# ChicyChen/LOCO-Edit

Hardware: AMD Instinct MI355X
Metric: edit-directions/sec (top-5 PMP-Jacobian SVD @256^2) + vT cos-sim vs ref (higher is better)
Workload: dtype bf16x3 (split-bf16 MFMA operands, fp32 accumulate + fp32 storage); 1 GPU; CelebA-HQ DDPM 256x256 top-5 local basis (l_eye-sized mask, L=2400), t=0.6T, 12 power iterations, one GPU; multi_gpu_form=single, probes_total=5, probes_per_gpu=5, kept=5, n_iter=12, mask_L=2400, weights=synthetic seed 0, streams=2

## Files before the change

### include/loco_hip_diag.h

```cpp
#ifndef LOCO_HIP_DIAG_H
#define LOCO_HIP_DIAG_H
#include "loco_hip.h"
#ifdef __cplusplus
extern "C" {
#endif

int  loco_bench_conv(loco_ctx* ctx, int32_t cin, int32_t cout, int32_t H, int32_t W, int32_t B, int32_t mode,
                     int32_t taps, int32_t tile, int32_t iters, float* ms_avg, void* stream);

typedef struct loco_conv_desc {
    int32_t struct_size;
    int32_t Cin, Cout, Hin, Win, B, taps;
    int32_t stride, upsample, zins, mode, cpg;
    int32_t transposed, accumulate, in_arena, pad;
    int32_t Cin2, cot_cpg;
    float   res_scale;
    int32_t st_cpg;
    const float *weight, *bias;
    const float *in, *bias2, *res;
    const float *prim, *sc, *sh, *mr, *gamma, *tst, *tc;
    const float *in2, *w2, *bias2nd;
    const float *cot_d, *cot_prim, *cot_sc, *cot_sh, *cot_mr, *cot_tc;
    float* out;
    const float *st_prim, *st_mr;
// ... 21 lines not shown
    const float *dq, *dk, *dv;
    float* out;
    const float* go;
    float *gq, *gk, *gv;
} loco_attn_desc;
int  loco_debug_attn(loco_ctx* ctx, const loco_attn_desc* desc, char* route, int64_t cap, void* stream);

typedef struct loco_norm_desc {
    int32_t struct_size;
    int32_t op, kind, act, B, C, HW, G, C1, ntA, ntB, accumulate;
    float   eps, base_scale;
    int64_t x_bs, d_bs, base_bs, out_bs, pbs_c, pbs_g, o_bs, t_bs;
    const float *x, *d, *base, *gamma, *beta, *ss_scale, *ss_shift, *sc, *sh, *mr, *tst, *partA, *partB;
    float *o_mr, *o_sc, *o_sh, *o_tst, *o_tc, *out;
} loco_norm_desc;
int  loco_debug_norm(loco_ctx* ctx, const loco_norm_desc* desc, void* stream);

typedef struct loco_gemm_prob {
    const float *A, *B, *A2, *B2, *bias, *colbias, *R;
    float* C;
    int64_t sam, sak, sab, sah;
    int64_t sbk, sbn, sbb, sbh;
    int64_t scm, scn, scb, sch;
    int64_t srb, sab2, sbb2;
    int64_t n_A, n_B, n_A2, n_B2, n_bias, n_colbias, n_R, n_C;
    int32_t M, N, K, batch, batch2;
    float   alpha, beta;
    int32_t pad_;
} loco_gemm_prob;
typedef struct loco_gemm_desc {
    int32_t struct_size;
    int32_t op, act, pad_;
    loco_gemm_prob p[2];
} loco_gemm_desc;
int  loco_debug_gemm(loco_ctx* ctx, const loco_gemm_desc* desc, char* route, int64_t cap, void* stream);

typedef struct loco_pointwise_desc {
    int32_t struct_size;
    int32_t op, kind, act, B, C, T, H, W, n, k, accumulate, cos_first;
    float   eps, scale, t, cv, ce;
    float   f[5];
    int32_t pad_;
    int64_t count, split, in_bs, out_bs, aux_bs, st_bs;
    const float *x, *y, *stats, *gamma, *beta, *base;
    const float *freq, *w0, *b0, *w1, *b1, *add, *add_in;
    const float *src[4];
    const uint8_t *mask, *mask2;
    float *out, *out2, *t_dev;
} loco_pointwise_desc;
int  loco_debug_pointwise(loco_ctx* ctx, const loco_pointwise_desc* desc, void* stream);

int64_t loco_debug_tensor(loco_ctx* ctx, const char* name, float* dst, int64_t cap, void* stream);

#ifdef __cplusplus
}
#endif
#endif
```

### loco-edit_amd/csrc/conv_bf16.hip

```cpp
#include "kernels.h"
#include <cstdio>
#include <cstdlib>

namespace loco {

enum : int { PR_BF16X3 = 0, PR_F16 = 1 };
template <int PR, int TAPS, int MODE> void launch_tile_b(const ConvArgs& a, hipStream_t st);
template <int PR, int MODE> void launch_kcat_b(const ConvArgs& a, hipStream_t st);
template <int PR, int MODE> void launch_pair_b(const ConvArgs& a, hipStream_t st);
void launch_conv_gemm(const ConvArgs& a, hipStream_t st);
template <int PR> void launch_poly_b(const ConvArgs& a, hipStream_t st);
template <int PR> void launch_poly_in_b(const ConvArgs& a, hipStream_t st);

template <int PR>
static void launch_lowp(const ConvArgs& a, int taps, hipStream_t st) {
#ifdef LOCO_DIAG
    if (a.cot_d && (taps != 1 || a.gemm || a.nsplit > 1 || a.Cin2 > 0 || (a.Cout % conv_bf16_tile_couts(a)) != 0 || a.st_kind == ST_TAN || a.st_kind == ST_COT)) {
        fprintf(stderr, "loco: ConvArgs::cot_d on a launch whose epilogue has no norm-cotangent term (taps %d, gemm %d, nsplit %d, Cout %d, st_kind %d)\n",
                taps, a.gemm, a.nsplit, a.Cout, a.st_kind);
        abort();
    }
#endif
    if constexpr (PR == PR_BF16X3) {
        if (taps == 1 && a.gemm) { launch_conv_gemm(a, st); return; }
    }
    if (taps == 9 && a.poly == 2) { launch_poly_in_b<PR>(a, st); return; }
    if (taps == 9 && a.poly) { launch_poly_b<PR>(a, st); return; }
    if (taps == 9 && a.Cin2 > 0) {
        if (a.mode == CM_GN_SILU) launch_kcat_b<PR, CM_GN_SILU>(a, st);
        else if (a.mode == CM_GN_GELU) launch_kcat_b<PR, CM_GN_GELU>(a, st);
        else launch_kcat_b<PR, CM_TAN_SILU>(a, st);
        return;
    }
    if constexpr (PR == PR_BF16X3) {
        if (taps == 9 && a.pair) {
            switch (a.mode) {
                case CM_NONE: launch_pair_b<PR, CM_NONE>(a, st); break;
                case CM_GN_SILU: launch_pair_b<PR, CM_GN_SILU>(a, st); break;
                case CM_TAN_SILU: launch_pair_b<PR, CM_TAN_SILU>(a, st); break;
                default: launch_pair_b<PR, CM_COT_SILU>(a, st); break;
            }
            return;
        }
    }
    if (taps == 9) {
        switch (a.mode) {
            case CM_NONE: launch_tile_b<PR, 9, CM_NONE>(a, st); break;
            case CM_GN_SILU: launch_tile_b<PR, 9, CM_GN_SILU>(a, st); break;
            case CM_GN_GELU: launch_tile_b<PR, 9, CM_GN_GELU>(a, st); break;
            case CM_TAN_SILU: launch_tile_b<PR, 9, CM_TAN_SILU>(a, st); break;
            case CM_COT_SILU: launch_tile_b<PR, 9, CM_COT_SILU>(a, st); break;
            default: launch_tile_b<PR, 9, CM_GN>(a, st); break;
        }
    } else {
        switch (a.mode) {
            case CM_NONE: launch_tile_b<PR, 1, CM_NONE>(a, st); break;
            default: launch_tile_b<PR, 1, CM_GN>(a, st); break;
        }
    }
}
void launch_conv_bf16x3(const ConvArgs& a, int taps, hipStream_t st) { launch_lowp<PR_BF16X3>(a, taps, st); }
void launch_conv_f16(const ConvArgs& a, int taps, hipStream_t st) { launch_lowp<PR_F16>(a, taps, st); }

}
```

### loco-edit_amd/csrc/conv_bf16_kernel.h

```cpp
#pragma once
#include "kernels.h"
#include <cstdlib>
#include <type_traits>

namespace loco {


typedef float f32x16 __attribute__((ext_vector_type(16)));
typedef float f32x4 __attribute__((ext_vector_type(4)));
typedef f32x4 f32x4_u __attribute__((aligned(4)));
typedef float f32x2 __attribute__((ext_vector_type(2)));
typedef f32x2 f32x2_u __attribute__((aligned(4)));
typedef __bf16 bf16x8 __attribute__((ext_vector_type(8)));
typedef _Float16 f16x8 __attribute__((ext_vector_type(8)));
typedef short s16x8 __attribute__((ext_vector_type(8)));

enum : int { PR_BF16X3 = 0, PR_F16 = 1 };

constexpr int BKC = 16;
constexpr bool LIVE_MASK = true;
constexpr bool EARLY_W = true;
constexpr int NDUMMY = 8;

__device__ __forceinline__ float sigmoidf2_(float y) { return __builtin_amdgcn_rcpf(1.0f + __expf(-y)); }
// ... 389 lines not shown
            o0[q] = f32x4{v0[0], v1[0], v0[1], v1[1]};
            o1[q] = f32x4{v0[2], v1[2], v0[3], v1[3]};
        }
        if (accu) {
            f32x4 r0[NP], r1[NP];
#pragma unroll
            for (int q = 0; q < NP; ++q) {
                const unsigned o = (unsigned)(ch0 + h * 32 + q * RSTEP + row0) * out_plane + pix0;
                r0[q] = *reinterpret_cast<const f32x4*>(ob + o);
                r1[q] = *reinterpret_cast<const f32x4*>(ob + o + 4);
            }
#pragma unroll
            for (int q = 0; q < NP; ++q) { o0[q] += r0[q]; o1[q] += r1[q]; }
        }
#pragma unroll
        for (int q = 0; q < NP; ++q) {
            const int co = ch0 + h * 32 + q * RSTEP + row0;
            const unsigned o = (unsigned)co * out_plane + pix0;
            float add = 0.f;
            if (a.bias) add += a.bias[co];
            if (b2) add += b2[co];
            o0[q] += add; o1[q] += add;
            __builtin_nontemporal_store(o0[q], reinterpret_cast<f32x4*>(ob + o));
            __builtin_nontemporal_store(o1[q], reinterpret_cast<f32x4*>(ob + o + 4));
            if (tan_st) {
                const f32x4 va = o0[q], vb = o1[q], xa = xs[q][0], xb = xs[q][1];
                av[(h * NP + q) * 2] = ((va[0] + va[1]) + (va[2] + va[3])) + ((vb[0] + vb[1]) + (vb[2] + vb[3]));
                av[(h * NP + q) * 2 + 1] = (fmaf(xa[0], va[0], xa[1] * va[1]) + fmaf(xa[2], va[2], xa[3] * va[3])) +
                                           (fmaf(xb[0], vb[0], xb[1] * vb[1]) + fmaf(xb[2], vb[2], xb[3] * vb[3]));
            }
        }
    }
    if (tan_st) {
        constexpr int STEPS = rs_steps(NV, 64), LEFT = NV >> STEPS;
        static_assert((NV & (NV - 1)) == 0, "row sums per lane");
        rs_reduce<NV, 1, 64>(av, lane);
        if (lane < (1 << STEPS)) {
            int base = 0;
#pragma unroll
            for (int sb = 0; sb < STEPS; ++sb) base += ((lane >> sb) & 1) * (NV >> (sb + 1));
            const int ntl = (a.Hout * a.Wout) / NT, ntile = 2 * ntl;
            float* const sp = a.st_part + (long)b * C * ntile * 2;
#pragma unroll
            for (int i = 0; i < LEFT; ++i) {
                const int idx = base + i, hq = idx >> 1;
                const int h = hq / NP, q = hq - h * NP;
                const int co = ch0 + h * 32 + q * RSTEP + row0;
                sp[((long)co * ntile + pa * ntl + tile_id) * 2 + (idx & 1)] = av[i];
            }
        }
    }
}

template <int PR, int TAPS, int WM, int WN, int TM, int TN, int MODE, int STG, int PHASE = 0>
__device__ __forceinline__ void conv_lowp_body(const ConvArgs& a, f32x16 (&acc)[TM][TN]) {
    constexpr int NTHR = WM * WN * 64;
    constexpr int HP = halo_pitch<PR>();
    constexpr int RB = rec_bytes<PR>();
    constexpr int NPC = RB / 16;
    constexpr int MT = WM * TM * 32;
    constexpr int NT = WN * TN * 32;
    constexpr bool POLY = (TAPS == 4 && STG == 0), PIN = (TAPS == 4 && STG == 1);
    static_assert(TAPS != 4 || POLY || PIN, "4-tap kernels: the two polyphase forms");
    static_assert(!PIN || (MODE == CM_NONE && PHASE == 0), "polyphase input form: raw");
    constexpr int KS = (TAPS == 9) ? 3 : (TAPS == 4 ? 2 : 1);
    constexpr int HK = (TAPS == 1) ? 1 : 3;
    constexpr int NTS = KS;
    constexpr int NROW = KS;
    static_assert(!POLY || (WM == 2 && TM == 2 && MODE == CM_NONE && PHASE == 0), "polyphase output form: 128 x 256 tile, raw vector staging");
    constexpr bool NEEDP = (MODE == CM_TAN_SILU || MODE == CM_COT_SILU);
    constexpr bool GEN = (STG == 1 || STG == 2);
    constexpr int NITEM = GEN ? (2 * max_halo(NT, TAPS, STG == 2) + NTHR - 1) / NTHR : 1;
    constexpr int WTOT = NTS * MT * NPC;
    constexpr int NWV = (WTOT + NTHR - 1) / NTHR;
    constexpr bool XPF = (TAPS == 9 && STG != 2);
    constexpr int NWB = XPF ? 3 : 2;
    constexpr bool DEEP1 = (TAPS == 1 && STG == 1 && !NEEDP);
    constexpr int DEEP_D = 4;

    extern __shared__ __attribute__((aligned(16))) unsigned char smem_b[];
#ifdef LOCO_DUAL_STAMP
#define LP_STAMP(i) do { if (threadIdx.x == 0 && PHASE == 0) reinterpret_cast<unsigned long long*>(a.partial)[blockIdx.x * 8 + (i)] = __builtin_amdgcn_s_memtime(); } while (0)
#else
#define LP_STAMP(i) do { } while (0)
#endif
    LP_STAMP(0);
    constexpr int WBYTES = NTS * MT * RB;
    unsigned char* const Wsb = smem_b;
    unsigned char* Hsb;
    unsigned char* Ws = smem_b;
    unsigned char* Hs = smem_b;

    const int tid = threadIdx.x;
    const int lane = tid & 63;
    const int wave = tid >> 6;
    const int l31 = lane & 31;
    const int khalf = lane >> 5;
    const int wm = wave / WN, wn = wave % WN;

    const int S = a.stride;
    const int TW = (TAPS == 1 && PHASE == 0 && a.stride == 1 && !a.upsample && !a.zins && (a.Wout & (a.Wout - 1)) == 0)
                       ? (a.Wout < NT ? a.Wout : NT) : (a.Wout < 32 ? a.Wout : 32);
    const int TH = NT / TW;
    const int tiles_x = a.Wout / TW;
    int tile_id, cot_id, zid;
    {
        const int ntile = (a.Hout * a.Wout) / NT, ncot = (a.Cout + MT - 1) / MT, Z = a.B * a.nsplit;
        const int NTC = ntile * ncot, L = blockIdx.x;
        int T = 0;
        if ((ntile & 7) == 0) {
            int q = L >> 3, q2, t8;
            idivmod_small(q, ncot, q2, cot_id);
            idivmod_small(q2, Z, t8, zid);
            tile_id = t8 * 8 + (L & 7);
        } else {
            if ((NTC & 7) == 0) { int q = L >> 3, t8; idivmod_small(q, Z, t8, zid); T = t8 * 8 + (L & 7); }
            else idivmod_small(L, Z, T, zid);
            idivmod_small(T, ntile, cot_id, tile_id);
        }
        tile_id = __builtin_amdgcn_readfirstlane(tile_id);
        cot_id = __builtin_amdgcn_readfirstlane(cot_id);
        zid = __builtin_amdgcn_readfirstlane(zid);
    }
    int ty0_, tx0_;
    idivmod_small(tile_id, tiles_x, ty0_, tx0_);
    const int oy0 = __builtin_amdgcn_readfirstlane(ty0_ * TH);
    const int ox0 = __builtin_amdgcn_readfirstlane(tx0_ * TW);
    const int co0 = cot_id * MT;
    int zb_, zs_;
    idivmod_small(zid, a.nsplit, zb_, zs_);
    const int b = __builtin_amdgcn_readfirstlane(zb_);
    const int split = __builtin_amdgcn_readfirstlane(zs_);

    if constexpr (XPF && PHASE != 2 && EARLY_W) {
        const int nchunks_ = (a.Cin + BKC - 1) / BKC;
        const int cps_ = __builtin_amdgcn_readfirstlane((nchunks_ + a.nsplit - 1) / a.nsplit);
        const int cbeg_ = split * cps_;
        const int cend_ = (cbeg_ + cps_ < nchunks_) ? cbeg_ + cps_ : nchunks_;
        if (cend_ > cbeg_) {
            typedef __attribute__((address_space(3))) unsigned char lds_u8_;
            typedef const __attribute__((address_space(1))) unsigned char glb_u8_;
            const int wpitch_ = (a.Cout + 31) & ~31;
            const unsigned char* wbase0 = reinterpret_cast<const unsigned char*>(a.wb) +
                                          (unsigned)(cbeg_ * TAPS) * ((unsigned)wpitch_ * (unsigned)RB);
#pragma unroll
            for (int st_ = 0; st_ < 2; ++st_)
#pragma unroll
                for (int i = 0; i < NWV; ++i) {
                    int e = tid + i * NTHR;
                    if (e >= WTOT) e = WTOT - 1;
                    const int tap = e / (MT * NPC), rem = e - tap * (MT * NPC);
                    int rec = co0 + rem / NPC;
                    if (rec >= wpitch_) rec = wpitch_ - 1;
                    const unsigned rel = (unsigned)(((st_ * NTS + tap) * wpitch_ + rec) * NPC + (rem % NPC)) * 16u;
                    const int e0 = wave * 64 + i * NTHR;
                    if ((WTOT % NTHR) == 0 || e0 < WTOT)
                        __builtin_amdgcn_global_load_lds((glb_u8_*)(wbase0 + rel), (lds_u8_*)(smem_b + st_ * WBYTES + e0 * 16), 16, 0, 0);
                }
        }
    }
    const int halo_w = (TW - 1) * S + HK;
    const int halo_h = (TH - 1) * S + HK;
    const int halo_sz = halo_h * halo_w;
    int pa_ = 0, pb_ = 0;
    if constexpr (POLY) {
        pa_ = __builtin_amdgcn_readfirstlane(idiv_small(cot_id, a.Cout >> 8));
        pb_ = __builtin_amdgcn_readfirstlane(wm);
    }
    int tap0 = pa_ * halo_w + pb_;
    const int HBYTES = (halo_sz + NDUMMY) * HP;
    Hsb = smem_b + NWB * WBYTES;

    const int LH = (a.upsample || a.zins) ? a.Hin * 2 : a.Hin;
    const int LW = (a.upsample || a.zins) ? a.Win * 2 : a.Win;
    const long in_plane = PIN ? 4L * a.Hin * a.Win : (long)a.Hin * a.Win;

    int ipos[NITEM], ioct[NITEM];
    unsigned ivoff[NITEM];
    bool ival[NITEM];
#pragma unroll
    for (int i = 0; i < NITEM; ++i) {
        int it = tid + i * NTHR;
        int oct, pos;
        idivmod_small(it, halo_sz, oct, pos);
        int off = -1;
// ... 645 lines not shown
                dma_w(cclamp(chunk + dc), r1, Wnxt);
                dma_live = true;
            }
            Ws = Wcur; Hs = Hcur;
            Frag f0, f1;
            load_frag(f0, row, 0);
            if (NTS > 1) load_frag(f1, row, 1);
            __builtin_amdgcn_sched_barrier(0);
            mma_frag(f0);
            __builtin_amdgcn_sched_barrier(0);
            if (NTS > 2) load_frag(f0, row, 2);
            __builtin_amdgcn_sched_barrier(0);
            if (NTS > 1) mma_frag(f1);
            if (st_part >= 0) { Hs = Hnxt; stage_h(cclamp(chunk + 1), st_part); Hs = Hcur; }
            if (MIDLOAD && ld_part >= 0) { pf_live = LIVE_MASK ? (ld_chunk <= clast) : true; prefetch_h(cclamp(ld_chunk), ld_part); pf_live = true; }
            if (NTS > 2) mma_frag(f0);
            __builtin_amdgcn_sched_barrier(0);
            if (MIDLOAD && ld_part >= 0) {
                asm volatile("s_waitcnt vmcnt(%0)" :: "n"(NLD) : "memory");
            } else {
                asm volatile("s_waitcnt vmcnt(0)" ::: "memory");
                if (!MIDLOAD && ld_part >= 0) { pf_live = LIVE_MASK ? (ld_chunk <= clast) : true; prefetch_h(cclamp(ld_chunk), ld_part); pf_live = true; }
            }
            stage_end();
        }
    }
    }

    }

    if constexpr (PHASE == 1) {
        asm volatile("s_waitcnt lgkmcnt(0)" ::: "memory");
        __builtin_amdgcn_s_barrier();
        return;
    }
    LP_STAMP(3);
    if constexpr (POLY) conv_lowp_epilogue_poly<WM, WN, TM, TN>(a, acc, smem_b, cot_id, pa_, oy0, ox0, TW, tile_id, b);
    else conv_lowp_epilogue<WM, WN, TM, TN, (TAPS == 1 && PHASE == 0) ? (EPI_COT1 | EPI_STATS) : EPI_STATS>(a, acc, smem_b, co0, oy0, ox0, TW, tile_id, b, split);
    LP_STAMP(4);
#undef LP_STAMP
}

constexpr int lowp_min_waves(int taps, int nthr) { return (taps == 1 && nthr <= 256) ? 2 : 1; }
template <int TAPS, int WM, int WN, int TM, int TN, int MODE, int STG>
__global__ __launch_bounds__(WM * WN * 64, lowp_min_waves(TAPS, WM * WN * 64)) void conv_mfma_bf16x3(ConvArgs a) {
    f32x16 acc[TM][TN];
    conv_lowp_body<PR_BF16X3, TAPS, WM, WN, TM, TN, MODE, STG>(a, acc);
}
template <int TAPS, int WM, int WN, int TM, int TN, int MODE, int STG>
__global__ __launch_bounds__(WM * WN * 64, lowp_min_waves(TAPS, WM * WN * 64)) void conv_mfma_f16(ConvArgs a) {
    f32x16 acc[TM][TN];
    conv_lowp_body<PR_F16, TAPS, WM, WN, TM, TN, MODE, STG>(a, acc);
}

template <int PR, int WM, int WN, int TM, int TN, int MODE>
__device__ __forceinline__ void conv_lowp_kcat(const ConvArgs& a) {
    f32x16 acc[TM][TN];
    conv_lowp_body<PR, 9, WM, WN, TM, TN, MODE, 0, 1>(a, acc);
    ConvArgs a2 = a;
    a2.in = a.in2; a2.in_bs = a.in2_bs; a2.Cin = a.Cin2; a2.wb = a.wb2; a2.mode = CM_NONE; a2.pad = 0; a2.in_padded = a.in2_padded;
    conv_lowp_body<PR, 1, WM, WN, TM, TN, CM_NONE, 1, 2>(a2, acc);
}
template <int WM, int WN, int TM, int TN, int MODE>
__global__ __launch_bounds__(WM * WN * 64) void conv_kcat_bf16x3(ConvArgs a) { conv_lowp_kcat<PR_BF16X3, WM, WN, TM, TN, MODE>(a); }
template <int WM, int WN, int TM, int TN, int MODE>
__global__ __launch_bounds__(WM * WN * 64) void conv_kcat_f16(ConvArgs a) { conv_lowp_kcat<PR_F16, WM, WN, TM, TN, MODE>(a); }

template <int PR, int TAPS, int WM, int WN, int TM, int TN, int MODE, int STG>
static void launch_one_b2(const ConvArgs& a, hipStream_t st) {
    constexpr int MT = WM * TM * 32, NT = WN * TN * 32;
    constexpr int KS = (TAPS == 9) ? 3 : (TAPS == 4 ? 2 : 1), HK = (TAPS == 1) ? 1 : 3;
    int TW = a.Wout < 32 ? a.Wout : 32;
    int TH = NT / TW;
    int halo_w = (TW - 1) * a.stride + HK, halo_h = (TH - 1) * a.stride + HK;
    const int nwb = (TAPS == 9 && STG != 2) ? 3 : 2;
    size_t lds = (size_t)nwb * KS * MT * rec_bytes<PR>() + 2 * ((size_t)halo_w * halo_h + NDUMMY) * halo_pitch<PR>();
    const size_t stage_bytes = (size_t)WM * 32 * NT * 4;
    if (lds < stage_bytes) lds = stage_bytes;
    dim3 grid(((a.Hout * a.Wout) / NT) * ((a.Cout + MT - 1) / MT) * a.B * a.nsplit);
    void (*kern)(ConvArgs);
    if constexpr (PR == PR_F16) kern = &conv_mfma_f16<TAPS, WM, WN, TM, TN, MODE, STG>;
    else kern = &conv_mfma_bf16x3<TAPS, WM, WN, TM, TN, MODE, STG>;
    if (lds > 64 * 1024) {
        static DeviceOnce once;
        if (first_on_device(once)) {
            (void)hipFuncSetAttribute(reinterpret_cast<const void*>(kern), hipFuncAttributeMaxDynamicSharedMemorySize,
                                      160 * 1024);
        }
    }
    hipLaunchKernelGGL(kern, grid, dim3(WM * WN * 64), lds, st, a);
}

template <int PR, int TAPS, int WM, int WN, int TM, int TN, int MODE>
static void launch_one_b(const ConvArgs& a, hipStream_t st) {
    const bool general = a.stride != 1 || a.upsample || a.zins || (a.Cin % BKC) != 0 || !a.in_padded;
    if constexpr (MODE == CM_NONE) {
        if (a.stride == 2) launch_one_b2<PR, TAPS, WM, WN, TM, TN, MODE, 2>(a, st);
        else if (TAPS == 9 && !general) launch_one_b2<PR, TAPS, WM, WN, TM, TN, MODE, 0>(a, st);
        else launch_one_b2<PR, TAPS, WM, WN, TM, TN, MODE, 1>(a, st);
        return;
    }
    if constexpr (MODE == CM_GN_SILU || MODE == CM_TAN_SILU || MODE == CM_GN_GELU) {
        if (general) { launch_one_b2<PR, TAPS, WM, WN, TM, TN, MODE, 1>(a, st); return; }
    }
    launch_one_b2<PR, TAPS, WM, WN, TM, TN, MODE, 0>(a, st);
}


template <int PR, int MODE>
void launch_kcat_b(const ConvArgs& a, hipStream_t st) {
    constexpr int WM = 2, WN = 4, TM = 2, TN = 2, MT = 128, NT = 256;
    const int TW = a.Wout < 32 ? a.Wout : 32, TH = NT / TW;
    size_t lds = (size_t)3 * 3 * MT * rec_bytes<PR>() + 2 * ((size_t)(TW + 2) * (TH + 2) + NDUMMY) * halo_pitch<PR>();
    dim3 grid(((a.Hout * a.Wout) / NT) * ((a.Cout + MT - 1) / MT) * a.B * a.nsplit);
    void (*kern)(ConvArgs);
    if constexpr (PR == PR_F16) kern = &conv_kcat_f16<WM, WN, TM, TN, MODE>;
    else kern = &conv_kcat_bf16x3<WM, WN, TM, TN, MODE>;
    static DeviceOnce once;
    if (first_on_device(once))
        (void)hipFuncSetAttribute(reinterpret_cast<const void*>(kern), hipFuncAttributeMaxDynamicSharedMemorySize, 160 * 1024);
    hipLaunchKernelGGL(kern, grid, dim3(WM * WN * 64), lds, st, a);
}

template <int PR>
void launch_poly_b(const ConvArgs& a, hipStream_t st) {
    ConvArgs v = a;
    v.Cout = 4 * a.Cout; v.Hout = a.Hin; v.Wout = a.Win;
    v.upsample = 0; v.zins = 0; v.stride = 1; v.pad = 1; v.nsplit = 1;
    launch_one_b2<PR, 4, 2, 4, 2, 2, CM_NONE, 0>(v, st);
}

template <int PR>
void launch_poly_in_b(const ConvArgs& a, hipStream_t st) {
    ConvArgs v = a;
    v.Cin = 4 * a.Cin; v.Hin = a.Hin / 2; v.Win = a.Win / 2;
    v.upsample = 0; v.zins = 0; v.stride = 1; v.pad = 1; v.nsplit = 1;
    launch_one_b2<PR, 4, 2, 4, 2, 2, CM_NONE, 1>(v, st);
}

template <int PR, int TAPS, int MODE>
void launch_tile_b(const ConvArgs& a, hipStream_t st) {
    switch (a.tile) {
        case 5:
            launch_one_b<PR, TAPS, 2, 4, 2, 2, MODE>(a, st);
            break;
        case 0: launch_one_b<PR, TAPS, 2, 2, 2, 2, MODE>(a, st); break;
        case 1: launch_one_b<PR, TAPS, 4, 1, 1, 2, MODE>(a, st); break;
        case 2: launch_one_b<PR, TAPS, 1, 4, 1, 1, MODE>(a, st); break;
        default: launch_one_b<PR, TAPS, 2, 2, 1, 1, MODE>(a, st); break;
    }
}


}
```

### loco-edit_amd/csrc/conv_plan.hip

```cpp
#include "kernels.h"
#include <cstdio>
#include <cstdlib>

namespace loco {

constexpr int BKC = 16;
constexpr int BKF = 8;

static const int kMT[6] = {128, 128, 32, 64, 128, 128}, kNT[6] = {128, 64, 128, 64, 256, 256};

static int env_int(const char* name, int dflt) {
    const char* e = getenv(name);
    return e ? atoi(e) : dflt;
}
static int pick_tile(int Cout, int HW) {
    if (HW >= 128) return Cout > 32 ? 0 : 2;
    return Cout > 64 ? 1 : 3;
}

static int conv_pick_nsplit(int Cin, int Cout, int Hout, int Wout, int B) {
    const int t = pick_tile(Cout, Hout * Wout);
    long blocks = (long)((Hout * Wout) / kNT[t]) * ((Cout + kMT[t] - 1) / kMT[t]) * B;
    int nchunks = (Cin + BKF - 1) / BKF;
    if (blocks >= 384 || nchunks < 8) return 1;
// ... 33 lines not shown
    static const bool on = env_int("LOCO_POLYPHASE", 1) != 0;
    if (!on || e.prec < 1 || taps != 9 || a.mode != CM_NONE || !(a.upsample || a.zins) || a.stride != 1) return false;
    if (!(e.prec == 2 ? a.wph : a.wpb) || !a.in_padded || a.res || a.Cin2 > 0 || a.cot_d) return false;
    if (a.upsample ? a.pad != 1 : (a.pad != 1 && a.pad != 2)) return false;
    if ((a.Cin % BKC) != 0 || (a.Cout % 128) != 0 || a.B < 2) return false;
    if (a.Hin * a.Win < 4096 || a.Win < 32 || (a.Win % 32) != 0 || (a.Hin % 8) != 0) return false;
    return a.Hout == 2 * a.Hin && a.Wout == 2 * a.Win;
}
static bool conv_poly_in_ok(const ConvEnv& e, const ConvArgs& a, int taps) {
    static const bool on = env_int("LOCO_POLYPHASE", 1) != 0;
    if (!on || e.prec < 1 || taps != 9 || a.mode != CM_NONE || !a.pool2 || a.upsample || a.zins || a.stride != 1 || a.pad != 1) return false;
    if (!(e.prec == 2 ? a.wqh : a.wqb) || a.res || a.bias2 || a.Cin2 > 0 || a.cot_d) return false;
    if ((a.Cin % BKC) != 0 || (a.Cout % 128) != 0 || a.B < 2 || ((a.Hin | a.Win) & 1)) return false;
    if (a.Hout * a.Wout < 4096 || a.Wout < 32 || (a.Wout % 32) != 0 || (a.Hout % 8) != 0) return false;
    return a.Hin == 2 * a.Hout && a.Win == 2 * a.Wout;
}

static int conv_bf16_pick_nsplit(int Cin, int Cout, int Hout, int Wout, int B, int chip_share, int taps, int lanes) {
    const int HW = Hout * Wout;
    int t = conv_bf16_pick_tile(Cout, HW, B, -1);
    if (t == 4) t = 5;
    if (taps == 1 && t == 5 && B >= 2 && HW <= kTile0MaxHW) t = 0;
    long blocks = (long)(HW / kNT[t]) * ((Cout + kMT[t] - 1) / kMT[t]) * B;
    int nchunks = (Cin + BKC - 1) / BKC;
    int target = chip_share > 1 ? 256 / chip_share : (lanes == 2 ? 240 : 256);
    if (target < 32) target = 32;
    if (blocks >= target / 2 || nchunks < 8) return 1;
    int want = (int)(target / blocks);
    int maxs = nchunks / 4;
    if (want > maxs) want = maxs;
    if (want > 32) want = 32;
    return want < 1 ? 1 : want;
}

static bool conv_lowp_can_kcat(const ConvArgs& a) {
    static const bool on = env_int("LOCO_KCAT", 1) != 0;
    return on && a.Cin2 > 0 && a.nsplit == 1 && bf16_tile_of(a) == 5 && a.stride == 1 && !a.upsample && !a.zins && a.pad == 1 &&
           (a.Cin % BKC) == 0 && (a.Cin2 % BKC) == 0 && a.in_padded &&
           (a.mode == CM_GN_SILU || a.mode == CM_GN_GELU || a.mode == CM_TAN_SILU);
}
static bool conv_lowp_can_fuse_stats(const ConvArgs& a) {
    return a.nsplit <= 1 && !a.gemm && (a.Cout % conv_bf16_tile_couts(a)) == 0;
}

static bool conv_pair_ok(const ConvArgs& a) {
    static const bool on = env_int("LOCO_CONV_PAIR", 1) != 0;
    if (!on || a.poly || a.Hout * a.Wout < 16384 || a.taps != 9 || a.Cin2 > 0 || a.nsplit != 1 || a.stride != 1 || a.upsample || a.zins ||
        a.pad != 1 || !a.in_padded || (a.Cin % (2 * BKC)) != 0 || (a.Cout % 128) != 0 || (a.Wout % 32) != 0 || (a.Hout % 8) != 0)
        return false;
    if (!(a.mode == CM_NONE || a.mode == CM_GN_SILU || a.mode == CM_TAN_SILU || a.mode == CM_COT_SILU)) return false;
    return a.tile == 5;
}

static ConvArgs conv_shift_batch(const ConvArgs& a, int nb) {
    ConvArgs t = a;
    t.B = a.B - nb;
    t.in += (long)nb * a.in_bs; t.out += (long)nb * a.out_bs;
    if (t.prim) t.prim += (long)nb * a.prim_bs;
    if (t.bias2) t.bias2 += (long)nb * a.bias2_bs;
    if (t.res) t.res += (long)nb * a.res_bs;
    if (t.sc) { t.sc += (long)nb * a.scsh_bs; t.sh += (long)nb * a.scsh_bs; }
    if (t.mr) t.mr += (long)nb * a.mr_bs;
    if (t.tst) t.tst += (long)nb * a.tst_bs;
    if (t.tc) t.tc += (long)nb * a.tc_bs;
    if (t.in2) t.in2 += (long)nb * a.in2_bs;
    if (t.cot_d) { t.cot_d += (long)nb * a.cot_d_bs; t.cot_tc += (long)nb * a.cot_tc_bs; }
    if (t.st_part) t.st_part += (long)nb * a.Cout * ((a.Hout * a.Wout) / conv_bf16_tile_pixels(a)) * 2;
    return t;
}

static void conv_gemm_plan(ConvArgs& a) {
    static const bool on = env_int("LOCO_CONV_GEMM", 1) != 0;
    a.gemm = 0;
    const long HW = (long)a.Hout * a.Wout;
    if (!on || a.stride != 1 || a.upsample || a.zins || (a.Cin % BKC) != 0 || a.Cin < 320 || (HW % 256) != 0 || (a.Wout % 16) != 0 ||
        a.Cout < 128 || !a.partial || a.Cin2 > 0 || !(a.mode == CM_NONE || a.mode == CM_GN) || a.cot_d)
        return;
    {
        const int TW = a.Wout < 32 ? a.Wout : 32;
        if ((256 % TW) != 0 || (a.Wout % TW) != 0 || (a.Hout % (256 / TW)) != 0) return;
    }
    static const int all_shapes = env_int("LOCO_GEMM_ALL", 0);
    if (!all_shapes && !(a.Cout >= 640 && (a.Cout >= 4 * a.Cin || a.Cin >= 2560))) return;
    const int pad256 = (a.Cout + 255) / 256 * 256;
    const int tm = (pad256 * 10 <= a.Cout * 11) ? 4 : 2;
    const int mt = 64 * tm;
    const long tiles = (HW / 256) * ((a.Cout + mt - 1) / mt) * a.B;
    const size_t rec_floats = (size_t)a.B * a.Cin * HW;
    int ns = 1;
    if (tiles < 192) {
        const int nchunks = a.Cin / BKC;
        ns = (int)((256 + tiles - 1) / tiles);
        if (ns > 8) ns = 8;
        while (ns > 1 && nchunks / ns < 8) --ns;
        while (ns > 1 && (size_t)ns * a.B * a.Cout * HW + rec_floats > a.partial_floats) --ns;
    }
    if ((ns > 1 ? (size_t)ns * a.B * a.Cout * HW : 0) + rec_floats > a.partial_floats) return;
    a.gemm = 1; a.gemm_tm = tm; a.nsplit = ns;
}

void conv_plan_family(ConvArgs& a, int prec) {
    if (prec == 1 && a.taps == 1) conv_gemm_plan(a);
}

void conv_plan_tile_pair(ConvArgs& a, int prec, int tile_override) {
    a.tile = tile_for(a, prec, tile_override);
// ... 59 lines not shown
}

ConvPlan plan_conv(const ConvEnv& e, const ConvArgs& a0, int taps, const StatAsk* q, const ConvArgs* sc) {
    ConvPlan p;
    ConvArgs a = a0;
    a.taps = taps;
    a.gemm = 0;
    a.poly = 0;
    if (a.pool2) {
        if (conv_poly_in_ok(e, a, taps)) a.poly = 2;
        else {
            p.pool_after = true; p.pool_out = a.out; p.pool_out_bs = a.out_bs; p.pool_acc = a.accumulate;
            a.out = a.pool_tmp; a.out_bs = a.pool_tmp_bs; a.Hout = a.Hin; a.Wout = a.Win; a.accumulate = 0; a.pool2 = 0;
        }
    }
    if (sc) {
        ConvArgs t = a;
        t.nsplit = e.prec >= 1 ? conv_bf16_pick_nsplit(a.Cin, a.Cout, a.Hout, a.Wout, a.B, e.chip_share, 9, e.lanes) : 2;
        t.in2 = sc->in; t.in2_bs = sc->in_bs; t.Cin2 = sc->Cin;
        const long per_probe = (long)((a.Hout * a.Wout) / 256) * ((a.Cout + 127) / 128);
        if (e.prec >= 1 && taps == 9 && !short_tail(per_probe, a.B) && !a.bias2 && conv_lowp_can_kcat(t)) {
            a.in2 = sc->in; a.in2_bs = sc->in_bs; a.Cin2 = sc->Cin; a.in2_padded = sc->in_padded;
            a.wb2 = e.prec == 2 ? sc->wh : sc->wb;
            a.bias2 = sc->bias; a.bias2_bs = 0;
            a.res = nullptr;
        } else {
            p.sc_first = true;
            a.res = sc->out; a.res_bs = sc->out_bs;
        }
    }
    if (e.prec == 2) a.wb = a.wh;
    a.no_deep = e.deep1 ? 0 : 1;
    a.nsplit = e.prec >= 1 ? conv_bf16_pick_nsplit(a.Cin, a.Cout, a.Hout, a.Wout, a.B, e.chip_share, taps, e.lanes)
                           : conv_pick_nsplit(a.Cin, a.Cout, a.Hout, a.Wout, a.B);
    if (a.cot_d) {
        ConvArgs t = a;
        t.tile = bf16_tile_of(t);
        const long per_probe = (long)((a.Hout * a.Wout) / conv_bf16_tile_pixels(t)) * ((a.Cout + 127) / 128);
        p.cot = e.prec >= 1 && taps == 1 && a.nsplit == 1 && !short_tail(per_probe, a.B) && conv_lowp_can_fuse_stats(t);
        if (!p.cot) { a.cot_d = nullptr; a.cot_d_bs = 0; a.cot_sx = nullptr; a.cot_tc = nullptr; a.cot_tc_bs = 0; }
    }
    while (a.nsplit > 1 && (size_t)a.nsplit * a.B * a.Cout * a.Hout * a.Wout > e.partial_floats) a.nsplit >>= 1;
    if (a.nsplit < 1) a.nsplit = 1;
    a.partial = e.partial;
    a.partial_floats = e.partial_floats;
    if (!a.poly && conv_poly_ok(e, a, taps)) a.poly = 1;
    if (a.poly == 1) { a.nsplit = 1; a.wb = e.prec == 2 ? a.wph : a.wpb; }
    if (a.poly == 2) { a.nsplit = 1; a.wb = e.prec == 2 ? a.wqh : a.wqb; }
    conv_plan_family(a, e.prec);
    a.tile = tile_for(a, e.prec, -1);
    int split = 1;
    const int tail = e.prec >= 1 && a.nsplit == 1 && a.B >= 2 && !a.gemm && !a.poly ? tail_split(a, e.partial_floats, &split) : 0;
    const bool want = q && q->kind != ST_NONE && e.prec >= 1 && e.fuse_stats;
    if (!tail) {
        p.l[0] = plan_launch(e, q, want, a, 0, a.B, &p.keep_ntile);
        return p;
    }
    const bool per_part = want && q->norm && (q->kind == ST_FWD || (e.fuse_lin && (a.Hout * a.Wout) % 4 == 0));
    p.stats_all = !per_part && q && q->kind != ST_NONE && q->norm;
    const StatAsk* ql = per_part ? q : nullptr;
    const int nb = a.B - tail;
    ConvArgs m = a, t = conv_shift_batch(a, nb);
    m.B = nb;
    t.nsplit = split;
    p.nl = 2;
    p.l[0] = plan_launch(e, ql, want, m, 0, a.B, &p.keep_ntile);
    p.l[1] = plan_launch(e, ql, want, t, nb, a.B, &p.keep_ntile);
    return p;
}

void polyphase_fold(int kind, int nin, int nout, const float* w, long so, long si, long st, float* out) {
    static const int sel[3][2][2][3] = {
        {{{1, 0, 0}, {0, 1, 1}}, {{1, 1, 0}, {0, 0, 1}}},
        {{{1, 0, 0}, {0, 0, 1}}, {{0, 1, 0}, {0, 0, 0}}},
        {{{0, 0, 0}, {0, 1, 0}}, {{1, 0, 0}, {0, 0, 1}}}};
    const long V = 4L * nout;
    for (int i = 0; i < nin; ++i)
        for (int pa = 0; pa < 2; ++pa)
            for (int pb = 0; pb < 2; ++pb)
                for (int ty = 0; ty < 2; ++ty)
                    for (int tx = 0; tx < 2; ++tx)
                        for (int o = 0; o < nout; ++o) {
                            double acc = 0.0;
                            for (int ky = 0; ky < 3; ++ky)
                                for (int kx = 0; kx < 3; ++kx)
                                    if (sel[kind][pa][ty][ky] && sel[kind][pb][tx][kx]) acc += (double)w[o * so + i * si + (3 * ky + kx) * st];
                            out[((long)i * 4 + 2 * ty + tx) * V + polyphase_vcout(nout, pa, pb, o)] = (float)acc;
                        }
}

void polyphase_fold_in(int nin, int nout, const float* w, long so, long si, long st, float* out, int noutP) {
    for (int p = 0; p < 2; ++p)
        for (int q = 0; q < 2; ++q)
            for (int i = 0; i < nin; ++i)
                for (int ty = 0; ty < 2; ++ty)
                    for (int tx = 0; tx < 2; ++tx) {
                        const int m = 2 * ty + 1 - p, n = 2 * tx + 1 - q;
                        for (int o = 0; o < nout; ++o) {
                            double acc = 0.0;
                            for (int a = 0; a < 2; ++a)
                                for (int b = 0; b < 2; ++b) {
                                    const int ky = m - a, kx = n - b;
                                    if (ky >= 0 && ky < 3 && kx >= 0 && kx < 3) acc += (double)w[o * so + i * si + (3 * ky + kx) * st];
                                }
                            out[((((long)(2 * p + q) * nin + i) * 4) + 2 * ty + tx) * noutP + o] = (float)acc;
                        }
                    }
}

const char* conv_variant_name(const ConvArgs& a, int taps, int prec) {
    static const char* tiles[6] = {"2,2,2,2", "4,1,1,2", "1,4,1,1", "2,2,1,1", "2,2,2,4", "2,4,2,2"};
    static char names[3][2][6][6][56];
    static char others[3][3][6][40];
    const int mode = (a.mode < 0 || a.mode > 5) ? 2 : a.mode;
    const char* other = nullptr;
    int k = 0, v = mode;
    if (prec && taps == 9 && a.poly) {
        static const char* pn[2][3] = {{"", "conv_mfma_bf16x3<4,2,4,2,2,0>", "conv_mfma_f16<4,2,4,2,2,0>"},
                                       {"", "conv_mfma_bf16x3<4,2,4,2,2,0>+pool", "conv_mfma_f16<4,2,4,2,2,0>+pool"}};
        return pn[a.poly == 2][prec];
    }
    if (prec && taps == 9 && a.Cin2 > 0) other = prec == 1 ? "conv_kcat_bf16x3<2,4,2,2,%d>" : "conv_kcat_f16<2,4,2,2,%d>";
    else if (prec == 1 && taps == 1 && a.gemm) { k = 1; other = "conv_gemm_bf16x3<%d>"; v = a.gemm_tm; }
    else if (prec == 1 && taps == 9 && a.pair) { k = 2; other = "conv_pair_bf16x3<%d>"; }
    if (other) {
        char* n = others[k][prec][v];
        if (!n[0]) snprintf(n, 40, other, v);
        return n;
    }
    int t = a.tile;
    if (t < 0 || t > 5) t = 0;
    int m = mode;
    if (taps != 9 && m != CM_NONE) m = CM_GN;
    if (!prec && m == CM_GN_GELU) m = CM_GN_SILU;
    char* n = names[prec][taps == 9 ? 0 : 1][t][m];
    static const char* kn[3] = {"conv_mfma_f32", "conv_mfma_bf16x3", "conv_mfma_f16"};
    if (!n[0]) snprintf(n, 56, "%s<%d,%s,%d>", kn[prec], taps, tiles[t], m);
    return n;
}

}
```

### loco-edit_amd/csrc/conv_plan_text.h

```cpp
#pragma once
#include "kernels.h"
#include <cstdio>
#include <string>

namespace loco {

inline const char* stat_route_name(int r) {
    static const char* names[5] = {"none", "epi", "splitk", "alone", "keep"};
    return r >= 0 && r < 5 ? names[r] : "?";
}

inline void conv_plan_text(const ConvPlan& p, int taps, int prec, std::string& out) {
    char line[384];
    for (int li = 0; li < p.nl; ++li) {
        const ConvLaunch& l = p.l[li];
        const ConvArgs& y = l.args;
        snprintf(line, sizeof(line),
                 "launch=%d part=0 kernel=%s tile=%d nsplit=%d B=%d s0=%d gemm=%d gemm_tm=%d pair=%d Cin2=%d sc_first=%d cot=%d "
                 "stats=%s ntile=%d\n",
                 li, conv_variant_name(y, taps, prec), y.tile, y.nsplit, y.B, l.s0, y.gemm, y.gemm ? y.gemm_tm : 0, y.pair, y.Cin2,
                 p.sc_first ? 1 : 0, p.cot ? 1 : 0, stat_route_name(l.stats), l.ntile);
        out += line;
    }
    snprintf(line, sizeof(line), "stats_all=%d keep_ntile=%d\n", p.stats_all ? 1 : 0, p.keep_ntile);
    out += line;
}

}
```

### loco-edit_amd/csrc/engine.hip

```cpp
#include <algorithm>
#include <array>
#include <cmath>
#include <cstdio>
#include <cstdlib>
#include <cstring>

#include "conv_plan_text.h"
#include "engine_internal.h"

using namespace loco;
using namespace loco::eng;

namespace loco {
namespace eng {

int upload(loco_ctx* c, float** dst, const std::vector<float>& h) {
    if (dalloc(c, dst, h.size() ? h.size() : 1)) return -1;
    HIPCHK(c, hipMemcpy(*dst, h.data(), h.size() * sizeof(float), hipMemcpyHostToDevice));
    return 0;
}

namespace {
struct Pass {
    loco_ctx* c;
    hipStream_t st;
    int B;
    float* arena;
    float* stats;
    TView T(int id) const { return tview(c, arena, id); }
};

static void drop_graphs(loco_ctx* c) {
    for (auto& kv : c->fwd_graphs) {
        if (kv.second.exec) (void)hipGraphExecDestroy(kv.second.exec);
        if (kv.second.graph) (void)hipGraphDestroy(kv.second.graph);
    }
    c->fwd_graphs.clear();
}
inline unsigned char* gemm_ws_get(loco_ctx* c, size_t need, hipStream_t st) {
    const int l = c->lane;
    if (c->gemm_ws_bytes[l] >= need) return c->gemm_ws[l];
    hipStreamCaptureStatus cs = hipStreamCaptureStatusNone;
    if (hipStreamIsCapturing(st, &cs) != hipSuccess || cs != hipStreamCaptureStatusNone) return nullptr;
    if (c->gemm_ws[l]) {
        (void)hipDeviceSynchronize();
        drop_graphs(c);
        (void)hipFree(c->gemm_ws[l]);
        c->bytes -= c->gemm_ws_bytes[l];
        c->gemm_ws[l] = nullptr; c->gemm_ws_bytes[l] = 0;
    }
    void* p = nullptr;
    if (hipMalloc(&p, need) != hipSuccess) { (void)hipGetLastError(); return nullptr; }
    c->gemm_ws[l] = static_cast<unsigned char*>(p); c->gemm_ws_bytes[l] = need; c->bytes += need;
    return c->gemm_ws[l];
}
inline void attn_note(loco_ctx* c, const char* kernel, const GemmArgs* g = nullptr) {
    if (!c->attn_log) return;
    char line[192];
    if (g) snprintf(line, sizeof(line), "kernel=%s M=%d N=%d K=%d batch=%d heads=%d kcat=%d\n", kernel, g->M, g->N, g->K, g->batch,
                    g->batch2 > 0 ? g->batch2 : 1, g->A2 ? 1 : 0);
    else snprintf(line, sizeof(line), "kernel=%s\n", kernel);
    *c->attn_log += line;
}
inline bool attn_gemm_rec(const loco_ctx* c, const GemmArgs& g) { return c->prec >= 1 && c->gemm_lowp && gemm_rec_eligible(g); }
inline void attn_gemm_f32(loco_ctx* c, const GemmArgs& g, hipStream_t st) { attn_note(c, "gemm_f32", &g); launch_gemm(g, st); }
inline void attn_gemm(loco_ctx* c, const GemmArgs& g, hipStream_t st) {
    if (attn_gemm_rec(c, g)) {
        if (unsigned char* ws = gemm_ws_get(c, gemm_rec_ws_bytes(g), st)) { attn_note(c, "gemm_rec", &g); launch_gemm_rec(g, ws, st); return; }
    }
    if (c->prec >= 1 && c->gemm_lowp && gemm_prefers_bf16x3(g)) { attn_note(c, "gemm_bf16x3", &g); launch_gemm_bf16x3(g, st); }
    else attn_gemm_f32(c, g, st);
}
inline void attn_gemm_pair(loco_ctx* c, const GemmArgs& g0, const GemmArgs& g1, hipStream_t st) {
    auto f32 = [&](const GemmArgs& g) { return !attn_gemm_rec(c, g) && !(c->prec >= 1 && c->gemm_lowp && gemm_prefers_bf16x3(g)); };
    if (!f32(g0) || !f32(g1)) { attn_gemm(c, g0, st); attn_gemm(c, g1, st); return; }
    attn_note(c, "gemm_f32", &g0); attn_note(c, "gemm_f32", &g1);
    launch_gemm_pair(g0, g1, st);
}
inline void attn_softmax_rows(loco_ctx* c, float* S, long rows, int T, hipStream_t st, int B, long bs) {
    attn_note(c, "softmax_rows"); launch_softmax_rows(S, rows, T, st, B, bs);
}
inline void attn_softmax_jac(loco_ctx* c, float* dS, const float* P, long rows, int T, float scale, hipStream_t st, int B, long bs) {
    attn_note(c, "softmax_jac"); launch_softmax_jac(dS, P, rows, T, rows, scale, st, B, bs);
}
}

NS nstats(const loco_ctx* c, float* base, const NormP& n) {
    NS s;
    s.sc = base + n.soff; s.sh = s.sc + n.C; s.mr = s.sh + n.C; s.tst = s.mr + 2 * c->cfg.gn_groups;
    s.tc = s.tst + 2 * c->cfg.gn_groups;
    return s;
}

static void stats_standalone(loco_ctx* c, const StatReq& rq, const float* x, long xbs, int B, int HW, int s0, hipStream_t st) {
    const NormP& n = *rq.n;
    const long SB = c->prog->stats_per_sample;
    const int G = c->cfg.gn_groups;
    if (rq.kind == ST_FWD) {
        NS s = nstats(c, rq.stats + (long)s0 * SB, n);
        launch_gn_stats(x, xbs, B, n.C, HW, G, eps_of(c, n), n.gamma, n.beta, s.mr, s.sc, s.sh, SB, c->red, st, rq.ss_scale,
                        rq.ss_shift);
    } else {
        NS sp = nstats(c, c->statsP, n);
        NS stt = nstats(c, rq.stats + (long)s0 * SB, n);
        launch_gn_tstats(x, xbs, rq.prim, 0, B, n.C, HW, G, sp.sc, sp.sh, sp.mr, 0, 0, rq.kind == ST_TAN ? 0 : 1, stt.tst,
                         stt.tc, SB, c->red, st, c->cfg.act);
    }
}

bool run_conv(loco_ctx* c, const ConvArgs& a0, int taps, hipStream_t st, const StatReq* rq, const ConvArgs* second) {
    const size_t span = (size_t)c->cfg.max_batch * c->prog->per_sample;
    auto padded = [&](const float* p) { return (p >= c->arenaP && p < c->arenaP + span) || (p >= c->arenaT && p < c->arenaT + span); };
    ConvArgs a = a0, sc;
    a.act = c->cfg.act;
    if (a.mode == CM_GN_SILU && c->cfg.act == ACT_GELU) a.mode = CM_GN_GELU;
    a.in_padded = padded(a.in);
    if (second) { sc = *second; sc.in_padded = padded(sc.in); }
    ConvEnv e;
    e.prec = c->prec; e.chip_share = c->chip_share; e.lanes = c->lanes_active; e.lane_s0 = c->lane_s0;
    e.partial = c->partial; e.partial_floats = c->partial_floats; e.stpart = c->stpart; e.stpart_floats = c->stpart_floats;
    e.fuse_stats = c->fuse_stats; e.fuse_lin = c->fuse_lin; e.deep1 = c->deep1; e.max_batch = c->cfg.max_batch;
    StatAsk q;
    if (rq) {
        q.kind = rq->kind; q.norm = rq->n != nullptr; q.prim = rq->prim; q.keep = rq->keep; q.keep_floats = rq->keep_floats;
        if (rq->n && rq->n->sx_off >= 0 && c->sxcache) q.sx = c->sxcache + rq->n->sx_off;
    }
    const ConvPlan p = plan_conv(e, a, taps, rq ? &q : nullptr, second ? &sc : nullptr);
    if (p.sc_first) run_conv(c, *second, 1, st);
    if (c->plan_log) conv_plan_text(p, taps, c->prec, *c->plan_log);
    if (rq && rq->kind != ST_NONE && rq->n) rq->n->ready = true;
    if (rq && rq->keep_ntile) *rq->keep_ntile = p.keep_ntile;
    const int HWo = a.Hout * a.Wout, Gn = c->cfg.gn_groups;
    const long SBs = c->prog->stats_per_sample;
    auto timed = [&](const char* name, double flops, const ConvArgs& y, auto&& launch) {
        loco_ctx::ProfRec r;
        if (c->prof_on) {
            r.name = name; r.flops = flops;
            r.cin = y.Cin; r.cout = y.Cout; r.h = y.Hout; r.b = y.B; r.ns = y.nsplit; r.mode = y.mode; r.taps = taps;
            r.e0 = c->next_event(); r.e1 = c->next_event();
            (void)hipEventRecord(r.e0, st);
        }
        launch();
        if (c->prof_on) { (void)hipEventRecord(r.e1, st); c->prof.push_back(r); }
    };
    for (int li = 0; li < p.nl; ++li) {
        const ConvLaunch& l = p.l[li];
        const ConvArgs& x = l.args;
        double flops = 2.0 * (x.Cin * taps + x.Cin2) * x.Cout * (double)x.Hout * x.Wout * x.B;
        if (x.zins) flops *= 0.25;
        if (x.poly == 2) flops *= 4.0;
        timed(c->prof_on ? conv_variant_name(x, taps, c->prec) : nullptr, flops, x, [&] {
            if (c->prec == 1) launch_conv_bf16x3(x, taps, st);
            else if (c->prec == 2) launch_conv_f16(x, taps, st);
            else launch_conv(x, taps, st);
        });
        if (x.nsplit > 1) {
            timed("conv_splitk_reduce", 0.0, x, [&] {
                if (l.stats != SR_SPLITK) { launch_conv_splitk_reduce(x, st); return; }
                const NormP& n = *rq->n;
                NS sp = nstats(c, c->statsP, n);
                NS so = nstats(c, rq->stats + (long)l.s0 * SBs, n);
                launch_conv_splitk_reduce_stats(x, rq->kind, Gn, eps_of(c, n), n.gamma, n.beta, so.mr, so.sc, so.sh, SBs, rq->ss_scale,
                                                rq->ss_shift, rq->prim, sp.sc, sp.sh, sp.mr, so.tst, so.tc, SBs, c->red, st);
            });
        }
        if (l.stats == SR_ALONE) stats_standalone(c, *rq, x.out, x.out_bs, x.B, HWo, l.s0, st);
        if (l.stats == SR_EPI) {
            const NormP& n = *rq->n;
            NS so = nstats(c, rq->stats + (long)l.s0 * SBs, n);
            if (rq->kind != ST_FWD) {
                NS sp = nstats(c, c->statsP, n);
                launch_gn_lin_fused_finalize(rq->kind, x.st_part, n.C, l.ntile, nullptr, 0, x.B, n.C, HWo, Gn, sp.mr, so.tst, so.tc,
                                             SBs, st);
            } else {
                launch_gn_fused_finalize(x.st_part, l.ntile, x.B, n.C, HWo, Gn, eps_of(c, n), n.gamma, n.beta, so.mr, so.sc, so.sh,
                                         SBs, rq->ss_scale, rq->ss_shift, st);
            }
        }
    }
    if (p.stats_all) stats_standalone(c, *rq, a.out, a.out_bs, a.B, HWo, 0, st);
    if (p.pool_after)
// ... 281 lines not shown
        attn_gemm_pair(c, attn_values(s, IMAGE, k, 0, SG, s.bS, gq, s.bq, s.HS, 0.f),
                       attn_keys(s, q, 0, s.HS, SG, s.bS, gk, s.bq), s.st);
        return;
    }
    attn_gemm(c, attn_keys(s, oG, s.bo, s.OS, SP, 0, gv, s.bq), s.st);
    if (s.Lt) attn_gemm_f32(c, attn_scores(s, TEXT, oG, s.bo, s.OS, s.vt, 0, SG, s.bS, 1.f, 0.f), s.st);
    attn_gemm(c, attn_scores(s, IMAGE, oG, s.bo, s.OS, v, 0, SG, s.bS, 1.f, 0.f), s.st);
    attn_softmax_jac(c, SG, SP, (long)s.NH * s.T, s.Tk, s.scale, s.st, s.B, s.bS);
    attn_gemm(c, attn_values(s, IMAGE, k, 0, SG, s.bS, gq, s.bq, s.HS, 0.f), s.st);
    if (s.Lt) attn_gemm_f32(c, attn_values(s, TEXT, s.kt, 0, SG, s.bS, gq, s.bq, s.HS, 1.f), s.st);
    attn_gemm(c, attn_keys(s, q, 0, s.HS, SG, s.bS, gk, s.bq), s.st);
}

}
}

namespace {

void lin1x1(loco_ctx* c, const ConvP& w, bool dgrad, const TView& in, const TView& out, int B, hipStream_t st,
            const float* bias = nullptr, const float* res = nullptr, const StatReq* rq = nullptr) {
    ConvArgs a = conv_args(in, w, dgrad, out, B, 1);
    a.bias = bias; a.res = res; a.res_bs = res ? out.bs : 0;
    run_conv(c, a, 1, st, rq);
}

void need_fwd_stats(const Pass& p, NormP& n, int tid, bool cat = false) {
    loco_ctx* c = p.c;
    if (!n.ready && !(cat && cat_fused_stats(c, n, tid, p.stats, p.B, p.st))) {
        const TView x = p.T(tid);
        NS s = nstats(c, p.stats, n);
        launch_gn_stats(x, x.bs, p.B, n.C, x.H * x.W, c->cfg.gn_groups, eps_of(c, n), n.gamma, n.beta, s.mr, s.sc, s.sh,
                        c->prog->stats_per_sample, c->red, p.st);
    }
    n.ready = false;
}

void lin_stats(const Pass& p, const NormP& n, int kind, const TView& d, const float* x) {
    loco_ctx* c = p.c;
    NS sp = nstats(c, c->statsP, n);
    NS stt = nstats(c, p.stats, n);
    launch_gn_tstats(d, d.bs, x, 0, p.B, n.C, d.H * d.W, c->cfg.gn_groups, sp.sc, sp.sh, sp.mr, 0, 0, kind, stt.tst,
                     stt.tc, c->prog->stats_per_sample, c->red, p.st, kind ? c->cfg.act : 0);
}
void need_tan_stats(const Pass& p, NormP& n, int tid, bool cat = false) {
    loco_ctx* c = p.c;
    if (!n.ready && !(cat && cat_fused_tstats(c, n, tid, p.B, p.st))) lin_stats(p, n, 0, p.T(tid), tview(c, c->arenaP, tid));
    n.ready = false;
}
void need_cot_stats(const Pass& p, NormP& n, const TView& d, const float* x) {
    if (!n.ready) lin_stats(p, n, 1, d, x);
    n.ready = false;
}
void gn_lin_apply(const Pass& p, const NormP& n, int kind, const TView& d, const float* x, const float* base, float* out,
                  int accumulate = 0, float base_scale = 1.0f) {
    loco_ctx* c = p.c;
    NS sp = nstats(c, c->statsP, n);
    NS stt = nstats(c, p.stats, n);
    launch_gn_apply(kind, d, d.bs, x, 0, base, base ? d.bs : 0, out, d.bs, accumulate, p.B, d.C, d.H * d.W, c->cfg.gn_groups,
                    sp.sc, sp.sh, sp.mr, 0, 0, stt.tst, c->prog->stats_per_sample, p.st, kind == 2 || kind == 5 ? c->cfg.act : 0,
                    base_scale);
}
void set_tan(loco_ctx* c, ConvArgs& a, const NormP& n, const float* prim) {
    NS sp = nstats(c, c->statsP, n);
    NS stt = nstats(c, c->statsT, n);
    a.mode = CM_TAN_SILU; a.prim = prim; a.prim_bs = 0;
    a.sc = sp.sc; a.sh = sp.sh; a.scsh_bs = 0; a.mr = sp.mr; a.mr_bs = 0; a.gamma_ = n.gamma;
    a.tst = stt.tst; a.tst_bs = c->prog->stats_per_sample; a.cpg = n.C / c->cfg.gn_groups;
    a.tc = stt.tc; a.tc_bs = c->prog->stats_per_sample;
    a.sx = (n.sx_off >= 0 && c->sxcache) ? c->sxcache + n.sx_off : nullptr;
}

constexpr size_t RED_BYTES = (size_t)4 << 20;

int forward_pass(loco_ctx* c, const float* x, float t, int B, float* arena, float* stats, hipStream_t st,
                 const float* t_ptr = nullptr, int op_hi = -1, const float* dh = nullptr) {
    const loco_unet_cfg& cfg = c->cfg;
    const Pass p{c, st, B, arena, stats};
    const long PS = c->prog->per_sample, SB = c->prog->stats_per_sample;
    auto T = [&](int id) { return p.T(id); };
    const TView xv = tview_in(x, c->prog->n_in, cfg.in_channels, cfg.resolution, cfg.resolution);
    clear_ready(c);
    auto next_fwd = [&](int tid) { return req_fwd_of(c, tid, stats); };
    auto gn_prologue = [&](ConvArgs& a, int mode, const NS& s) { a.mode = mode; a.sc = s.sc; a.sh = s.sh; a.scsh_bs = SB; };
    if (cfg.arch < 2) {
        launch_temb(t, cfg.ch, cfg.ch * 4, c->wts->freq, c->wts->td0w, c->wts->td0b, c->wts->td1w, c->wts->td1b, c->tact, st, cfg.arch == 1,
                    c->has_cond ? c->cond_add : nullptr, t_ptr, cfg.act, c->has_tcond ? c->cond_in : nullptr);
        launch_temb_proj(c->tact, cfg.ch * 4, c->wts->tp_w, c->wts->tp_b, (int)c->wts->tproj_total, c->tproj, st);
    }
    const int op_end = op_hi >= 0 ? op_hi : (int)c->ops.size() - 1;
    for (int oi = 0; oi <= op_end; ++oi) {
        Op& op = c->ops[oi];
        const Tens& to = c->tens[op.out];
        switch (op.kind) {
            case OP_CONV_IN: case OP_CONV: {
                ConvArgs a = conv_args(op.kind == OP_CONV_IN ? xv : T(op.in), op.conv, false, T(op.out), B, op.ksize);
                a.bias = op.conv.bias;
                const StatReq rq = next_fwd(op.out);
                run_conv(c, a, op.ksize == 1 ? 1 : 9, st, &rq);
                break;
            }
            case OP_RES: {
                const Tens& ti = c->tens[op.in];
                need_fwd_stats(p, op.n1, op.in, true);
                NS s1 = nstats(c, stats, op.n1);
                if (op.updown == 1) {
                    launch_gn_apply(4, nullptr, 0, T(op.in), PS, nullptr, 0, T(op.a1), PS, 0, B, ti.C, ti.H * ti.W,
                                    cfg.gn_groups, s1.sc, s1.sh, s1.mr, SB, SB, nullptr, 0, st, cfg.act);
                    launch_pool2x2_sum(T(op.a1), PS, T(op.ap), PS, 0, B, ti.C, to.H, to.W, st, 0.25f);
                    launch_pool2x2_sum(T(op.in), PS, T(op.xu), PS, 0, B, ti.C, to.H, to.W, st, 0.25f);
                } else if (op.updown == 2) {
                    launch_upsample2x(T(op.in), PS, T(op.xu), PS, 0, 1.0f, B, ti.C, ti.H, ti.W, st);
                }
                ConvArgs a = conv_args(op.updown == 1 ? T(op.ap) : T(op.in), op.c1, false, T(op.h1), B, 3);
// ... 47 lines not shown
                    lin1x1(c, op.xproj, false, T(op.xo), T(op.out), B, st, op.xproj.bias, T(op.xmid), &rqx);
                }
                break;
            }
            case OP_XFMR: {
                if (!c->has_ctx) { c->err = "this architecture has cross-attention stages: call loco_set_context first"; return -1; }
                const int C = to.C, HW = to.H * to.W;
                auto X = [&](int i) { return T(op.xt[i]); };
                need_fwd_stats(p, op.n1, op.in);
                {
                    ConvArgs a = conv_args(T(op.in), op.pj_in, false, X(X_H0), B, 1);
                    a.bias = op.pj_in.bias;
                    gn_prologue(a, CM_GN, nstats(c, stats, op.n1));
                    run_conv(c, a, 1, st);
                }
                const XA xa = xa_of(c, op, B, st);
                launch_ln_fwd(X(X_H0), PS, B, C, HW, op.lng[0], op.lnb[0], 1e-5f, X(X_A1), PS, X(X_LN1), PS, st);
                lin1x1(c, op.qkvc, false, X(X_A1), X(X_QKV), B, st);
                attn_forward(attn_of(c, op, B, st, arena, PS));
                lin1x1(c, op.to_out1, false, X(X_O), X(X_H1), B, st, op.to_out1.bias, X(X_H0));
                launch_ln_fwd(X(X_H1), PS, B, C, HW, op.lng[1], op.lnb[1], 1e-5f, X(X_A2), PS, X(X_LN2), PS, st);
                lin1x1(c, op.xqc, false, X(X_A2), X(X_XQ), B, st);
                xa_forward(xa, X(X_XQ), X(X_XS), X(X_XO));
                lin1x1(c, op.to_out2, false, X(X_XO), X(X_H2), B, st, op.to_out2.bias, X(X_H1));
                launch_ln_fwd(X(X_H2), PS, B, C, HW, op.lng[2], op.lnb[2], 1e-5f, X(X_A3), PS, X(X_LN3), PS, st);
                lin1x1(c, op.ff1, false, X(X_A3), X(X_F), B, st, op.ff1.bias);
                launch_geglu(0, X(X_F), PS, nullptr, B, 4L * C * HW, X(X_GG), PS, st);
                lin1x1(c, op.ff2, false, X(X_GG), X(X_H3), B, st, op.ff2.bias, X(X_H2));
                const StatReq rq = next_fwd(op.out);
                lin1x1(c, op.pj_out, false, X(X_H3), T(op.out), B, st, op.pj_out.bias, T(op.in), &rq);
                break;
            }
            case OP_DOWN: case OP_UP: {
                ConvArgs a = conv_args(T(op.in), op.conv, false, T(op.out), B, 3);
                a.bias = op.conv.bias;
                if (op.kind == OP_DOWN) { a.stride = 2; a.pad = op.sym_down ? 1 : 0; } else { a.upsample = 1; }
                const StatReq rq = next_fwd(op.out);
                run_conv(c, a, 9, st, &rq);
                break;
            }
            case OP_OUT: {
                need_fwd_stats(p, op.n1, op.in);
                ConvArgs a = conv_args(T(op.in), op.conv, false, T(op.out), B, 3);
                a.bias = op.conv.bias;
                gn_prologue(a, CM_GN_SILU, nstats(c, stats, op.n1));
                run_conv(c, a, 9, st);
                break;
            }
        }
    }
    return 0;
}

int tangent_pass(loco_ctx* c, const float* V, int B, hipStream_t st, int op_lo = 0, int op_hi = -1) {
    const loco_unet_cfg& cfg = c->cfg;
    const long PS = c->prog->per_sample;
    const Pass p{c, st, B, c->arenaT, c->statsT};
    auto TP = [&](int id) { return tview(c, c->arenaP, id); };
    auto TT = [&](int id) { return p.T(id); };
    const TView Vv = tview_in(V, c->prog->n_in, cfg.in_channels, cfg.resolution, cfg.resolution);
    clear_ready(c);
    auto next_tan = [&](int tid) {
        StatReq r = req_lin(c, ST_TAN, consumer_norm(c, tid), TP(tid));
        Tens& t = c->tens[tid];
        if (t.cat_of >= 0 && t.keep && c->fuse_lin) {
            r.kind = ST_TAN; r.stats = c->statsT; r.prim = TP(tid);
            r.keep = t.keep; r.keep_floats = t.keep_floats; r.keep_ntile = &t.keep_ntile;
        }
        return r;
    };
    const int op_end = op_hi >= 0 ? op_hi : (int)c->ops.size() - 1;
    for (int oi = op_lo; oi <= op_end; ++oi) {
        Op& op = c->ops[oi];
        const Tens& to = c->tens[op.out];
        switch (op.kind) {
            case OP_CONV_IN: case OP_CONV: {
                const ConvArgs a = conv_args(op.kind == OP_CONV_IN ? Vv : TT(op.in), op.conv, false, TT(op.out), B, op.ksize);
                const StatReq rq = next_tan(op.out);
                run_conv(c, a, op.ksize == 1 ? 1 : 9, st, &rq);
                break;
            }
            case OP_RES: {
                const Tens& ti = c->tens[op.in];
                need_tan_stats(p, op.n1, op.in, true);
                if (op.updown == 1) {
                    gn_lin_apply(p, op.n1, 5, TT(op.in), TP(op.in), nullptr, TT(op.a1));
                    launch_pool2x2_sum(TT(op.a1), PS, TT(op.ap), PS, 0, B, ti.C, to.H, to.W, st, 0.25f);
                    launch_pool2x2_sum(TT(op.in), PS, TT(op.xu), PS, 0, B, ti.C, to.H, to.W, st, 0.25f);
                } else if (op.updown == 2) {
                    launch_upsample2x(TT(op.in), PS, TT(op.xu), PS, 0, 1.0f, B, ti.C, ti.H, ti.W, st);
                }
                ConvArgs a = conv_args(op.updown == 1 ? TT(op.ap) : TT(op.in), op.c1, false, TT(op.h1), B, 3);
                if (op.updown != 1) { set_tan(c, a, op.n1, TP(op.in)); a.upsample = op.updown == 2; }
                {
                    const StatReq rq2 = req_lin(c, ST_TAN, &op.n2, TP(op.h1));
                    run_conv(c, a, 9, st, &rq2);
                    op.n2.ready = false;
                }
                const TView xin = op.updown ? TT(op.xu) : TT(op.in);
                ConvArgs n{};
                if (op.has_nin) n = conv_args(xin, op.nin, false, TT(op.out), B, 1);
                ConvArgs b = conv_args(TT(op.h1), op.c2, false, TT(op.out), B, 3);
                b.res = xin; b.res_bs = PS;
                b.res_scale = op.has_nin ? 1.f : c->prog->res_scale;
                set_tan(c, b, op.n2, TP(op.h1));
                const StatReq rq = next_tan(op.out);
// ... 6 lines not shown
                gn_lin_apply(p, op.n1, 1, TT(op.in), TP(op.in), nullptr, TT(op.hn));
                lin1x1(c, op.qkvc, false, TT(op.hn), TT(op.qkv), B, st);
                attn_tangent(attn_of(c, op, B, st));
                {
                    const StatReq rq = next_tan(so);
                    lin1x1(c, op.proj, false, TT(op.o), TT(so), B, st, nullptr, TT(op.in), &rq);
                }
                if (op.has_x) {
                    const XA x = xa_of(c, op, B, st);
                    need_tan_stats(p, op.nx, op.xmid);
                    gn_lin_apply(p, op.nx, 1, TT(op.xmid), TP(op.xmid), nullptr, TT(op.xhn));
                    lin1x1(c, op.xqc, false, TT(op.xhn), TT(op.xq), B, st);
                    xa_linear(x, TT(op.xq), op.xK, op.xV, TP(op.xS), TT(op.xS), TT(op.xo));
                    const StatReq rqx = next_tan(op.out);
                    lin1x1(c, op.xproj, false, TT(op.xo), TT(op.out), B, st, nullptr, TT(op.xmid), &rqx);
                }
                break;
            }
            case OP_XFMR: {
                const int C = to.C, HW = to.H * to.W;
                auto XP = [&](int i) { return TP(op.xt[i]); };
                auto XT_ = [&](int i) { return TT(op.xt[i]); };
                need_tan_stats(p, op.n1, op.in);
                gn_lin_apply(p, op.n1, 1, TT(op.in), TP(op.in), nullptr, XT_(X_G0));
                lin1x1(c, op.pj_in, false, XT_(X_G0), XT_(X_H0), B, st);
                const XA xa = xa_of(c, op, B, st);
                launch_ln_tan(XT_(X_H0), PS, XP(X_H0), XP(X_LN1), B, C, HW, op.lng[0], XT_(X_A1), PS, st);
                lin1x1(c, op.qkvc, false, XT_(X_A1), XT_(X_QKV), B, st);
                attn_tangent(attn_of(c, op, B, st));
                lin1x1(c, op.to_out1, false, XT_(X_O), XT_(X_H1), B, st, nullptr, XT_(X_H0));
                launch_ln_tan(XT_(X_H1), PS, XP(X_H1), XP(X_LN2), B, C, HW, op.lng[1], XT_(X_A2), PS, st);
                lin1x1(c, op.xqc, false, XT_(X_A2), XT_(X_XQ), B, st);
                xa_linear(xa, XT_(X_XQ), op.xK, op.xV, XP(X_XS), XT_(X_XS), XT_(X_XO));
                lin1x1(c, op.to_out2, false, XT_(X_XO), XT_(X_H2), B, st, nullptr, XT_(X_H1));
                launch_ln_tan(XT_(X_H2), PS, XP(X_H2), XP(X_LN3), B, C, HW, op.lng[2], XT_(X_A3), PS, st);
                lin1x1(c, op.ff1, false, XT_(X_A3), XT_(X_F), B, st);
                launch_geglu(1, XT_(X_F), PS, XP(X_F), B, 4L * C * HW, XT_(X_GG), PS, st);
                lin1x1(c, op.ff2, false, XT_(X_GG), XT_(X_H3), B, st, nullptr, XT_(X_H2));
                const StatReq rq = next_tan(op.out);
                lin1x1(c, op.pj_out, false, XT_(X_H3), TT(op.out), B, st, nullptr, TT(op.in), &rq);
                break;
            }
            case OP_DOWN: case OP_UP: {
                ConvArgs a = conv_args(TT(op.in), op.conv, false, TT(op.out), B, 3);
                if (op.kind == OP_DOWN) { a.stride = 2; a.pad = op.sym_down ? 1 : 0; } else { a.upsample = 1; }
                const StatReq rq = next_tan(op.out);
                run_conv(c, a, 9, st, &rq);
                break;
            }
            case OP_OUT: {
                need_tan_stats(p, op.n1, op.in);
                ConvArgs a = conv_args(TT(op.in), op.conv, false, TT(op.out), B, 3);
                set_tan(c, a, op.n1, TP(op.in));
                run_conv(c, a, 9, st);
                break;
            }
        }
    }
    return 0;
}

int cotangent_pass(loco_ctx* c, const float* ge, const float* gx0, float* Aout, int B, hipStream_t st, int op_lo = 0,
                   int op_hi = -1) {
    const loco_unet_cfg& cfg = c->cfg;
    const long PS = c->prog->per_sample;
    const Pass p{c, st, B, c->arenaT, c->statsT};
    auto TP = [&](int id) { return tview(c, c->arenaP, id); };
    auto TG = [&](int id) { return p.T(id); };
    auto GO = [&](const Op& o) {
        const Tens& t = c->tens[o.out];
        return o.out == c->prog->eps_t ? tview_in(ge, c->prog->n_out, t.C, t.H, t.W) : TG(o.out);
    };
    const TView Av{Aout, c->prog->n_in, cfg.in_channels, cfg.resolution, cfg.resolution};
    clear_ready(c);
    for (int oi = op_hi >= 0 ? op_hi : (int)c->ops.size() - 1; oi >= op_lo; --oi) {
        Op& op = c->ops[oi];
        const Tens& to = c->tens[op.out];
        const int acc = op.in_is_skip ? 1 : 0;
        switch (op.kind) {
            case OP_OUT: {
                const ConvArgs a = conv_args(GO(op), op.conv, true, TG(op.a1), B, 3);
                {
                    const StatReq rq = req_lin(c, ST_COT, &op.n1, TP(op.in));
                    run_conv(c, a, 9, st, &rq);
                    op.n1.ready = false;
                }
                gn_lin_apply(p, op.n1, 2, TG(op.a1), TP(op.in), nullptr, TG(op.in));
                break;
            }
            case OP_UP: {
                ConvArgs a = conv_args(TG(op.out), op.conv, true, TG(op.in), B, 3);
                a.pool2 = 1; a.pool_tmp = TG(op.up); a.pool_tmp_bs = PS;
                run_conv(c, a, 9, st);
                break;
            }
            case OP_DOWN: {
                ConvArgs a = conv_args(TG(op.out), op.conv, true, TG(op.in), B, 3);
                a.zins = 1; a.pad = op.sym_down ? 1 : 2; a.accumulate = acc;
                run_conv(c, a, 9, st);
                break;
            }
            case OP_RES: {
                const Tens& ti = c->tens[op.in];
                {
                    const ConvArgs a = conv_args(TG(op.out), op.c2, true, TG(op.h1), B, 3);
                    const StatReq rq2 = req_lin(c, ST_COT, &op.n2, TP(op.h1));
                    run_conv(c, a, 9, st, &rq2);
                    op.n2.ready = false;
                }
                ConvArgs b = conv_args(TG(op.h1), op.c1, true, TG(op.updown == 0 ? op.a1 : op.updown == 1 ? op.ap : op.xu), B, 3);
                set_tan(c, b, op.n2, TP(op.h1));
                b.mode = CM_COT_SILU;
                if (op.updown == 0) {
                    const StatReq rq1 = req_lin(c, ST_COT, &op.n1, TP(op.in));
                    run_conv(c, b, 9, st, &rq1);
                } else if (op.updown == 1) {
                    run_conv(c, b, 9, st);
                    launch_upsample2x(TG(op.ap), PS, TG(op.a1), PS, 0, 0.25f, B, ti.C, to.H, to.W, st);
                } else {
                    run_conv(c, b, 9, st);
                    launch_pool2x2_sum(TG(op.xu), PS, TG(op.a1), PS, 0, B, ti.C, ti.H, ti.W, st);
                }
                need_cot_stats(p, op.n1, TG(op.a1), TP(op.in));
                bool cot_in_epilogue = false;
                if (op.has_nin) {
                    ConvArgs n = conv_args(TG(op.out), op.nin, true, TG(op.in), B, 1);
                    n.accumulate = acc;
                    if (op.updown == 0 && c->prec >= 1 && c->fuse_cot && op.n1.sx_off >= 0 && c->sxcache) {
                        n.cot_d = TG(op.a1); n.cot_d_bs = PS; n.cot_sx = c->sxcache + op.n1.sx_off;
                        n.cot_tc = nstats(c, c->statsT, op.n1).tc; n.cot_tc_bs = c->prog->stats_per_sample;
                    }
                    cot_in_epilogue = run_conv(c, n, 1, st);
                }
                if (op.updown == 0) {
                    if (cot_in_epilogue) {  }
                    else if (op.has_nin) gn_lin_apply(p, op.n1, 2, TG(op.a1), TP(op.in), nullptr, TG(op.in), 1);
                    else
                        gn_lin_apply(p, op.n1, 2, TG(op.a1), TP(op.in), TG(op.out), TG(op.in), acc, c->prog->res_scale);
                } else {
                    gn_lin_apply(p, op.n1, 2, TG(op.a1), TP(op.in), nullptr, TG(op.in), acc);
// ... 133 lines not shown
    c->cfg = *cfg;
    c->prog = std::move(prog);
    const size_t MB = (size_t)cfg->max_batch;
    {
        float *p0 = nullptr, *p1 = nullptr;
        if (dalloc(c, &p0, MB * c->prog->per_sample + 128) || dalloc(c, &p1, MB * c->prog->per_sample + 128)) return -1;
        c->arenaP = p0 + 64; c->arenaT = p1 + 64;
    }
    if (dalloc(c, &c->statsP, MB * c->prog->stats_per_sample) || dalloc(c, &c->statsT, MB * c->prog->stats_per_sample)) return -1;
    if (dalloc(c, &c->red, RED_BYTES) || dalloc(c, &c->red2, RED_BYTES)) return -1;
    if (alloc_state(c)) return -1;
    {
        c->stpart_floats = MB * (size_t)(c->prog->max_tensor / 64 + 1) * 2;
        if (dalloc(c, &c->stpart, c->stpart_floats) || dalloc(c, &c->stpart2, c->stpart_floats)) return -1;
        const char* e = getenv("LOCO_FUSE_STATS");
        c->fuse_stats = !(e && atoi(e) == 0);
        e = getenv("LOCO_FUSE_LIN");
        c->fuse_lin = !(e && atoi(e) == 0);
        e = getenv("LOCO_FUSE_COT");
        c->fuse_cot = !(e && atoi(e) == 0) && cfg->act == ACT_SILU;
        e = getenv("LOCO_DEEP1");
        c->deep1 = !(e && atoi(e) == 0);
        e = getenv("LOCO_FUSE_XATTN");
        c->fuse_xattn = !(e && atoi(e) == 0);
        const char* fa = getenv("LOCO_FLASH_ATTN");
        c->flash_attn = !(fa && atoi(fa) == 0);
        if (dalloc(c, &c->attn_delta, MB * (size_t)c->prog->attn_dmax)) return -1;
    }
    c->partial_floats = (size_t)64 << 20;
    if (dalloc(c, &c->partial, c->partial_floats)) return -1;
    if (dalloc(c, &c->xin_buf, MB * c->prog->n_in) || dalloc(c, &c->t_dev, 4)) return -1;
    if (dalloc(c, &c->eps_buf, MB * c->prog->n_out) || dalloc(c, &c->gx0, MB * c->prog->n_in) || dalloc(c, &c->ge, MB * c->prog->n_out))
        return -1;
    c->n_ws = std::max((long)c->prog->n_in, (long)c->prog->n_h);
    if (dalloc(c, &c->tmpA, (size_t)64 * c->n_ws)) return -1;
    if (dalloc(c, &c->G, 64 * 64) || dalloc(c, &c->Q, 64 * 64) || dalloc(c, &c->W, SOLVER_W_GATE + 1)) return -1;
    {
        size_t nblk = ((size_t)c->n_ws + 255) / 256;
        if (dalloc(c, &c->gscratch, nblk * 64 * 64 + 4096)) return -1;
    }
    if (dalloc(c, &c->kry[0], KRY_STATE) || dalloc(c, &c->kry[1], KRY_STATE)) return -1;
    if (dalloc(c, &c->alphas, 256) || dalloc(c, &c->cond_add, (size_t)cfg->ch * 4)) return -1;
    if (dalloc(c, &c->cond_in, (size_t)cfg->ch)) return -1;
    {
        float2* sx0 = nullptr;
        if (dalloc(c, &sx0, (size_t)c->prog->sx_total + 64)) return -1;
        c->sxcache = sx0 + 32;
    }
    {
        const char* e = getenv("LOCO_PRECISION");
        c->prec = (e && std::string(e) == "f32") ? 0 : (e && std::string(e) == "f16") ? 2 : 1;
    }
    if (dalloc(c, &c->mask2, (size_t)c->prog->n_out)) return -1;
    if (dalloc(c, &c->mask, (size_t)c->prog->n_out) || dalloc(c, &c->mask_idx, (size_t)c->prog->n_out) ||
        dalloc(c, &c->mask_L_dev, 4)) return -1;
    HIPCHK(c, hipEventCreate(&c->ev0));
    HIPCHK(c, hipEventCreate(&c->ev1));
    {
        const char* e = getenv("LOCO_STREAMS");
        c->n_streams = (e && atoi(e) == 2) ? 2 : 1;
        HIPCHK(c, hipStreamCreateWithFlags(&c->st2, hipStreamNonBlocking));
        HIPCHK(c, hipStreamCreateWithFlags(&c->cap_st, hipStreamNonBlocking));
        const char* gl = getenv("LOCO_GEMM_LOWP");
        if (gl) c->gemm_lowp = atoi(gl) != 0;
        const char* gr = getenv("LOCO_GRAPH");
        c->graph_on = gr && atoi(gr) == 1;
        HIPCHK(c, hipEventCreateWithFlags(&c->ev_fork, hipEventDisableTiming));
        HIPCHK(c, hipEventCreateWithFlags(&c->ev_join, hipEventDisableTiming));
    }
    return 0;
}

}

extern "C" {

const char* loco_version(void) { return "loco_hip 0.2 (gfx950; conv arithmetic: f32 MFMA | bf16x3 split-bf16 MFMA | f16 MFMA)"; }

int loco_device_count(void) {
    int n = 0;
    if (hipGetDeviceCount(&n) != hipSuccess) return 0;
    return n;
}

int loco_create(const loco_unet_cfg* cfg, loco_ctx** out) {
    if (!cfg || !out) return -2;
    loco_ctx* c = new loco_ctx();
    *out = c;
    if (cfg->struct_size != (int32_t)sizeof(loco_unet_cfg)) {
        c->err = "loco_unet_cfg.struct_size = " + std::to_string(cfg->struct_size) + ", this library expects " +
                 std::to_string(sizeof(loco_unet_cfg)) + " (binding and library built from different headers)";
        return -2;
    }
    auto prog = std::make_shared<Program>();
    if (const int rc = build_program(*cfg, prog.get(), &c->err)) return rc;
    for (const ParamDecl& d : prog->params) c->params[d.name].shape = d.shape;
    c->wts = std::make_shared<Weights>();
    c->wts->op.resize(prog->ops.size());
    return create_ctx(c, cfg, std::move(prog));
}

int loco_fork(loco_ctx* parent, int32_t max_batch, loco_ctx** out) {
    if (!parent || !out) return -2;
    *out = nullptr;
    if (finalize_params(parent)) return -3;
    loco_ctx* root = parent->weights_of ? parent->weights_of : parent;
// ... 196 lines not shown
                    void* stream) {
    return loco_pmp_primal_tap(c, x, t, at, mask, use_et, 0, stream);
}

static int pmp_primal_at(loco_ctx* c, const float* x, float t, float at, const uint8_t* mask, int32_t use_et, int32_t tap, const float* dh,
                         void* stream) {
    if (tap < 0 || tap > 2) { c->err = "loco_pmp_primal_tap: tap must be 0 (x_t -> x0 / eps), 1 (encoder, x_t -> h) or 2 (decoder, h -> eps)"; return -2; }
    if (tap && tap_refuse(c, "loco_pmp_primal_tap")) return -2;
    if (tap == 1 && mask) { c->err = "loco_pmp_primal_tap: the encoder tap (x_t -> h) takes no mask: h has no pixel positions to select"; return -2; }
    if (finalize_params(c)) return -3;
    if (dh) {
        const Op& op = c->ops[c->prog->h_last_op];
        if (op.kind != OP_RES || op.has_nin || op.updown) { c->err = "loco_pmp_primal_tap_dh: the tap op is not an identity-shortcut ResBlock"; return -2; }
    }
    if (tap == 1) use_et = 1;
    if (c->prog->n_out != c->prog->n_in && !use_et) {
        c->err = "loco_pmp_primal: a network whose output size differs from its input has no x0 combination; use_et = 1 "
                 "(raw network Jacobian)";
        return -2;
    }
    hipStream_t st = (hipStream_t)stream;
    const int op_lo = tap == 2 ? c->prog->h_last_op + 1 : 0, op_hi = tap == 1 ? c->prog->h_last_op : (int)c->ops.size() - 1;
    if (forward_pass(c, x, t, 1, c->arenaP, c->statsP, st, nullptr, tap == 1 ? op_hi : -1, dh)) return -1;
    c->primal_B = 1;
    if (c->prec >= 1) {
        for (int oi = op_lo; oi <= op_hi; ++oi) {
            Op& op = c->ops[oi];
            if (op.kind != OP_RES && op.kind != OP_OUT) continue;
            const Tens& ti = c->tens[op.in];
            const int HW = ti.H * ti.W, G = c->cfg.gn_groups;
            NS s1 = nstats(c, c->statsP, op.n1);
            launch_gn_cache(c->arenaP + ti.off, op.n1.C, HW, op.n1.C / G, s1.sc, s1.sh, s1.mr,
                            c->sxcache + op.n1.sx_off, st, c->cfg.act);
            if (op.kind == OP_RES) {
                const Tens& th = c->tens[op.h1];
                NS s2 = nstats(c, c->statsP, op.n2);
                launch_gn_cache(c->arenaP + th.off, op.n2.C, th.H * th.W, op.n2.C / G, s2.sc, s2.sh, s2.mr,
                                c->sxcache + op.n2.sx_off, st, c->cfg.act);
            }
        }
    }
    if (use_et) { c->p_cv = 0.f; c->p_ce = 1.f; }
    else { c->p_cv = 1.0f / std::sqrt(at); c->p_ce = -std::sqrt(1.0f - at) / std::sqrt(at); }
    if (tap == 2) c->p_cv = 0.f;
    c->tap = tap;
    c->has_mask = (mask != nullptr);
    c->has_mask2 = false;
    c->mask_L = tap == 1 ? c->prog->n_h : c->prog->n_out;
    if (mask) {
        HIPCHK(c, hipMemcpyAsync(c->mask, mask, (size_t)c->prog->n_out, hipMemcpyDeviceToDevice, st));
        launch_mask_compact(c->mask, c->prog->n_out, c->mask_idx, c->mask_L_dev, st);
        c->mask_L = -1;
        c->mask_stream = st;
    }
    HIPCHK(c, hipGetLastError());
    c->primal_ok = true;
    return 0;
}

int loco_pmp_primal_tap(loco_ctx* c, const float* x, float t, float at, const uint8_t* mask, int32_t use_et, int32_t tap,
                        void* stream) {
    if (!c) return -2;
    return pmp_primal_at(c, x, t, at, mask, use_et, tap, nullptr, stream);
}

int loco_pmp_primal_tap_dh(loco_ctx* c, const float* x, float t, float at, const uint8_t* mask, int32_t use_et, const float* dh,
                           void* stream) {
    if (!c) return -2;
    if (tap_refuse(c, "loco_pmp_primal_tap_dh")) return -2;
    return pmp_primal_at(c, x, t, at, mask, use_et, 2, dh, stream);
}

int loco_pmp_primal_eps(loco_ctx* c, float* eps, void* stream) {
    if (!c) return -2;
    if (!eps) { c->err = "loco_pmp_primal_eps: eps is NULL"; return -2; }
    if (!c->primal_ok) { c->err = "loco_pmp_primal has not been called"; return -2; }
    if (c->tap == 1) { c->err = "loco_pmp_primal_eps: the encoder tap's primal stops at h, there is no network output to hand out"; return -2; }
    launch_copy(c->arenaP + c->tens[c->prog->eps_t].off, c->prog->per_sample, eps, c->prog->n_out, 0, 1, c->prog->n_out, (hipStream_t)stream);
    HIPCHK(c, hipGetLastError());
    return 0;
}

int loco_pmp_set_second_mask(loco_ctx* c, const uint8_t* mask2, int32_t from_row, void* stream) {
    if (!c) return -2;
    if (!c->primal_ok) { c->err = "loco_pmp_primal has not been called"; return -2; }
    if (!mask2) { c->has_mask2 = false; return 0; }
    if (!c->has_mask) { c->err = "a second mask needs a first one (loco_pmp_primal with mask)"; return -2; }
    if (from_row < 0) { c->err = "from_row must be >= 0"; return -2; }
    HIPCHK(c, hipMemcpyAsync(c->mask2, mask2, (size_t)c->prog->n_out, hipMemcpyDeviceToDevice, (hipStream_t)stream));
    c->has_mask2 = true;
    c->mask2_from = from_row;
    return 0;
}

int loco_pmp_jvp(loco_ctx* c, const float* V, int32_t k, float* U, void* stream) {
    if (!c) return -2;
    if (!c->primal_ok) { c->err = "loco_pmp_primal has not been called"; return -2; }
    hipStream_t st = (hipStream_t)stream;
    const int MB = c->cfg.max_batch;
    for (int b0 = 0; b0 < k; b0 += MB) {
        int B = (k - b0 < MB) ? k - b0 : MB;
        int rc = run_lanes(c, B, st, [&](int s0, int nb, hipStream_t ls) -> int {
            const Program& P = *c->prog;
            if (c->tap == 1) {
                if (tangent_pass(c, V + (long)(b0 + s0) * P.n_in, nb, ls, 0, P.h_last_op)) return -1;
                launch_copy(c->arenaT + c->tens[P.h_t].off, P.per_sample, U + (long)(b0 + s0) * P.n_h, P.n_h, 0, nb, P.n_h, ls);
// ... 505 lines not shown
```

### loco-edit_amd/csrc/engine_diag.hip

```cpp
#include <cmath>
#include <cstdio>
#include <cstdlib>
#include <cstring>
#include <initializer_list>

#include "../../include/loco_hip_diag.h"
#include "conv_plan_text.h"
#include "engine_internal.h"

using namespace loco;
using namespace loco::eng;

static void release_since(loco_ctx* c, hipStream_t st, size_t owned0, size_t bytes0) {
    (void)hipStreamSynchronize(st);
    while (c->owned.size() > owned0) { (void)hipFree(c->owned.back()); c->owned.pop_back(); }
    c->bytes = bytes0;
}

__global__ void diag_fill_records(unsigned char* rec, long nrec, int wpitch, unsigned seed, float scale) {
    const long r = (long)blockIdx.x * 256 + threadIdx.x;
    if (r >= nrec) return;
    const int idx = (int)(r % wpitch);
    unsigned short hi[16], lo[16];
    for (int k = 0; k < 16; ++k) {
// ... 678 lines not shown
            break;
        }
        default:
            if (gemm_pair_grouped(g[0], g[1])) { note("gemm_f32_pair", g[0], 0, 0); note("gemm_f32_pair", g[1], 0, 0); }
            else { note(f32_name[gemm_f32_variant(g[0])], g[0], 0, 0); note(f32_name[gemm_f32_variant(g[1])], g[1], 0, 0); }
            launch_gemm_pair(g[0], g[1], st);
            break;
    }
    hipError_t he = hipStreamSynchronize(st);
    if (ws) (void)hipFree(ws);
    if (he == hipSuccess) he = hipGetLastError();
    if (he != hipSuccess) { c->err = std::string("debug_gemm: ") + hipGetErrorString(he); return -1; }
    if (route && cap > 0) {
        if ((int64_t)text.size() + 1 > cap) { c->err = "debug_gemm: route buffer too small"; return -4; }
        std::memcpy(route, text.c_str(), text.size() + 1);
    }
    return 0;
}

int64_t loco_debug_tensor(loco_ctx* c, const char* name, float* dst, int64_t cap, void* stream) {
    if (!c) return -2;
    std::string nm(name);
    if (nm == "bench_out") {
        if (!c->bench_out) { c->err = "no loco_bench_conv yet"; return -3; }
        int64_t cnt = cap < c->bench_out_count ? cap : c->bench_out_count;
        HIPCHK(c, hipMemcpyAsync(dst, c->bench_out, (size_t)cnt * sizeof(float), hipMemcpyDeviceToDevice, (hipStream_t)stream));
        return cnt;
    }
    if (nm == "workspace") {
        int64_t cnt = cap < (int64_t)c->partial_floats ? cap : (int64_t)c->partial_floats;
        HIPCHK(c, hipMemcpyAsync(dst, c->partial, (size_t)cnt * sizeof(float), hipMemcpyDeviceToDevice, (hipStream_t)stream));
        return cnt;
    }
    int arena = 0;
    if (nm.rfind("T:", 0) == 0) { arena = 1; nm = nm.substr(2); }
    bool want_h1 = false;
    if (nm.rfind("h1:", 0) == 0) { want_h1 = true; nm = nm.substr(3); }
    for (auto& op : c->ops) {
        if (op.name != nm) continue;
        int id = want_h1 ? op.h1 : op.out;
        if (id < 0) return -3;
        const Tens& t = c->tens[id];
        int64_t cnt = (int64_t)t.C * t.H * t.W;
        int B = arena ? 1 : (c->primal_B > 0 ? c->primal_B : 1);
        if (cnt * B > cap) { c->err = "debug buffer too small"; return -4; }
        float* base = (arena ? c->arenaT : c->arenaP) + t.off;
        launch_copy(base, c->prog->per_sample, dst, cnt, 0, B, cnt, (hipStream_t)stream);
        return cnt * B;
    }
    c->err = "no such op: " + nm;
    return -3;
}

}
```

### loco-edit_amd/csrc/engine_internal.h

```cpp
#pragma once
#include <hip/hip_runtime.h>

#include <cstdint>
#include <cstring>
#include <map>
#include <memory>
#include <string>
#include <vector>

#include "../../include/loco_hip.h"
#include "kernels.h"
#include "program.h"

#define HIPCHK(ctx, call)                                                                    \
    do {                                                                                     \
        hipError_t e_ = (call);                                                              \
        if (e_ != hipSuccess) {                                                              \
            (ctx)->err = std::string(#call) + ": " + hipGetErrorString(e_);                  \
            return -1;                                                                       \
        }                                                                                    \
    } while (0)

namespace loco {
namespace eng {
// ... 65 lines not shown

    float *arenaP = nullptr, *arenaT = nullptr;
    float *statsP = nullptr, *statsT = nullptr;
    double* red = nullptr;
    bool fuse_cot = true;
    float *stpart = nullptr, *stpart2 = nullptr;
    size_t stpart_floats = 0;
    bool fuse_stats = true;
    bool fuse_xattn = true;
    bool deep1 = true;
    bool flash_attn = true;
    float* attn_delta = nullptr;
    float* partial = nullptr;
    size_t partial_floats = 0;
    const float* bench_out = nullptr; int64_t bench_out_count = 0;
    std::string* plan_log = nullptr;
    std::string* attn_log = nullptr;
    float *tact = nullptr, *tproj = nullptr;
    float* eps_buf = nullptr;
    float* gx0 = nullptr;
    float* ge = nullptr;
    float* tmpA = nullptr;
    double *G = nullptr, *Q = nullptr, *W = nullptr, *gscratch = nullptr;
    double* kry[2] = {nullptr, nullptr};
    int kry_m[2] = {0, 0}, kry_k[2] = {0, 0};
    float* alphas = nullptr;
    float* ctx_colbias = nullptr;
    bool has_ctx = false;
    float* ctx_G = nullptr;
    bool ctx_G_first = false;
    float* cond_add = nullptr;
    float* ctx_norm = nullptr;
    bool has_cond = false;
    float* cond_in = nullptr;
    bool has_tcond = false;
    float2* sxcache = nullptr;
    int prec = 0;
    std::vector<float*> owned;
    size_t bytes = 0;

    bool primal_ok = false;
    float p_cv = 0.f, p_ce = 0.f;
    int tap = 0;
    long n_ws = 0;
    uint8_t* mask = nullptr;
    bool has_mask = false;
    uint8_t* mask2 = nullptr;
    bool has_mask2 = false;
    int mask2_from = 0;
    int* mask_idx = nullptr;
    int* mask_L_dev = nullptr;
    long mask_L = 0;
    hipStream_t mask_stream = nullptr;
    int primal_B = 0;
    hipEvent_t ev0 = nullptr, ev1 = nullptr;
    int n_streams = 1;
    hipStream_t st2 = nullptr;
    hipStream_t st2_user = nullptr;
    hipEvent_t ev_fork = nullptr, ev_join = nullptr;
    double* red2 = nullptr;
    struct FwdGraph { hipGraph_t graph = nullptr; hipGraphExec_t exec = nullptr; int calls = 0; };
    std::map<int, FwdGraph> fwd_graphs;
    bool graph_on = false;
    bool gemm_lowp = true;
    unsigned char* gemm_ws[2] = {nullptr, nullptr}; size_t gemm_ws_bytes[2] = {0, 0}; int lane = 0;
    loco_ctx* weights_of = nullptr;
    int forks = 0;
    bool zombie = false;
    bool fuse_lin = true;
    int lanes_active = 1;
    int lane_s0 = 0;
    int chip_share = 1;
    hipStream_t cap_st = nullptr;
    float* xin_buf = nullptr;
    float* t_dev = nullptr;
    bool prof_on = false;
    struct ProfRec { const char* name; double flops; hipEvent_t e0, e1; int cin, cout, h, b, ns, mode, taps; };
    bool prof_shapes = false;
    std::vector<ProfRec> prof;
    std::vector<hipEvent_t> ev_pool;
    size_t ev_used = 0;
    hipEvent_t next_event() {
        if (ev_used == ev_pool.size()) {
            hipEvent_t e; (void)hipEventCreate(&e); ev_pool.push_back(e);
        }
        return ev_pool[ev_used++];
    }
};

namespace loco {
namespace eng {

template <typename T>
int dalloc(loco_ctx* c, T** p, size_t count) {
    void* q = nullptr;
    HIPCHK(c, hipMalloc(&q, count * sizeof(T)));
    *p = reinterpret_cast<T*>(q);
    c->owned.push_back(reinterpret_cast<float*>(q));
    c->bytes += count * sizeof(T);
    return 0;
}

inline float eps_of(const loco_ctx* c, const NormP& n) { return n.eps > 0.f ? n.eps : c->cfg.gn_eps; }
int upload(loco_ctx* c, float** dst, const std::vector<float>& h);

int make_conv(loco_ctx* c, const std::vector<const HostParam*>& ws, const std::vector<const HostParam*>& bs,
              ConvP* out, int row_limit = -1, int poly_kind = -1, bool poly_dgrad = false);
int make_conv1(loco_ctx* c, const std::string& name, ConvP* out, int row_limit = -1, int poly_kind = -1, bool poly_dgrad = false);
int make_conv1_scaled(loco_ctx* c, const std::string& name, ConvP* out, float s);
int make_norm(loco_ctx* c, const std::string& name, NormW* n);
int bind_weights(loco_ctx* c);
int finalize_params(loco_ctx* c);

struct NS { float *sc, *sh, *mr, *tst, *tc; };
NS nstats(const loco_ctx* c, float* base, const NormP& n);

struct StatReq {
    int kind = ST_NONE;
    NormP* n = nullptr;
    float* stats = nullptr;
    const float* prim = nullptr;
    const float* ss_scale = nullptr; const float* ss_shift = nullptr;
    float* keep = nullptr; size_t keep_floats = 0; int* keep_ntile = nullptr;
};

inline void conv_defaults(ConvArgs& a) {
    std::memset(&a, 0, sizeof(a));
    a.stride = 1; a.pad = 1; a.nsplit = 1; a.mode = CM_NONE; a.res_scale = 1.f;
}
inline void setw(ConvArgs& a, const ConvP& p, bool dgrad) {
    a.w = dgrad ? p.wd : p.wf;
    a.wb = dgrad ? (const void*)p.wbd : (const void*)p.wbf;
    a.wh = dgrad ? (const void*)p.whd : (const void*)p.whf;
    const bool folded = p.wpb && p.poly_dgrad == dgrad;
    a.wpb = folded ? p.wpb : nullptr;
    a.wph = folded ? p.wph : nullptr;
    a.wqb = dgrad ? p.wqb : nullptr;
    a.wqh = dgrad ? p.wqh : nullptr;
}

struct TView {
    float* p; long bs; int C, H, W;
    operator float*() const { return p; }
};
inline TView tview(const loco_ctx* c, float* arena, int id) {
    const Tens& t = c->tens[id];
    return {arena + t.off, c->prog->per_sample, t.C, t.H, t.W};
}
inline TView tview_in(const float* p, long bs, int C, int H, int W) { return {const_cast<float*>(p), bs, C, H, W}; }
inline ConvArgs conv_args(const TView& in, const ConvP& w, bool dgrad, const TView& out, int B, int ksize) {
    ConvArgs a; conv_defaults(a);
    a.in = in.p; a.in_bs = in.bs; a.Cin = in.C; a.Hin = in.H; a.Win = in.W;
    setw(a, w, dgrad);
    a.out = out.p; a.out_bs = out.bs; a.Cout = out.C; a.Hout = out.H; a.Wout = out.W; a.B = B;
    if (ksize == 1) a.pad = 0;
    return a;
}
bool run_conv(loco_ctx* c, const ConvArgs& a0, int taps, hipStream_t st, const StatReq* rq = nullptr,
              const ConvArgs* second = nullptr);

struct XA {
    loco_ctx* c; hipStream_t st; int B; int C, T, NH, CH, L, Lp;
    float scale;
    const float *xK, *xV;
    const float* colbias;
    long xs, ss;
};
void xa_forward(const XA& x, const float* Xq, float* P, float* O);
void xa_linear(const XA& x, const float* X, const float* K1, const float* K2, float* P, float* S, float* O);
int xa_context_grad(const XA& x, const Op& op, const float* go, const float* q, const float* P, float* S);

struct Attn {
    loco_ctx* c; hipStream_t st;
    int B, T, NH, CH, Lt, Tk;
    long HS, SS, OS, KS;
    float scale;
    bool pair;
    const float *q, *k, *v, *P, *o;
    float *tq, *tk, *tv, *tS, *to;
    long bq, bS, bo;
    const float *kt, *vt;
    const float* colbias;
    float* delta;
    unsigned char* ws; size_t ws_bytes;
    bool flash() const {
        return c->flash_attn && c->prec >= 1 && (Lt ? attn_flash_text_supported(T, CH, Lt) : attn_flash_supported(T, CH));
    }
};
AttnFlashArgs attn_flash_args(const Attn& s);
void attn_forward(const Attn& s);
void attn_tangent(const Attn& s);
void attn_cotangent(const Attn& s);

}
}
```

### loco-edit_amd/csrc/kernels.h

```cpp
#pragma once
#include <hip/hip_runtime.h>
#include <stdint.h>

namespace loco {

struct DeviceOnce { bool seen[64] = {}; };
inline bool first_on_device(DeviceOnce& f) {
    int d = 0;
    (void)hipGetDevice(&d);
    d &= 63;
    if (f.seen[d]) return false;
    f.seen[d] = true;
    return true;
}


enum ConvMode : int {
    CM_NONE = 0,
    CM_GN_SILU = 1,
    CM_GN = 2,
    CM_TAN_SILU = 3,
    CM_COT_SILU = 4,
    CM_GN_GELU = 5,
};
// ... 3 lines not shown
    return y * (1.0f / (1.0f + __expf(-y)));
}
__device__ __forceinline__ float act_der(float y, int act) {
    if (act == ACT_GELU) return 0.5f * (1.0f + erff(y * 0.70710678118654752f)) + y * 0.39894228040143268f * __expf(-0.5f * y * y);
    const float sg = 1.0f / (1.0f + __expf(-y));
    return sg * (1.0f + y * (1.0f - sg));
}

enum StatKind : int { ST_NONE = 0, ST_FWD = 1, ST_TAN = 2, ST_COT = 3 };

struct ConvArgs {
    const float* in; long in_bs; int Cin, Hin, Win;
    const float* prim; long prim_bs;
    const float* w;
    const void* wb;
    const void* wh;
    const float2* sx;
    float* out; long out_bs; int Cout, Hout, Wout;
    const float* bias;
    const float* bias2; long bias2_bs;
    const float* res; long res_bs;
    const float* sc; const float* sh; long scsh_bs;
    const float* mr; long mr_bs;
    const float* gamma_;
    const float* tst; long tst_bs;
    const float* tc; long tc_bs;
    int cpg;
    int mode;
    int stride;
    int pad;
    int upsample;
    int zins;
    int in_padded;
    int accumulate;
    int nsplit;
    int taps;
    int no_deep;
    float* partial;
    int B;
    float* st_part; int st_kind;
    const float* st_x; const float2* st_sx;
    const float* in2; long in2_bs; int Cin2; int in2_padded;
    const void* wb2;
    const float* cot_d; long cot_d_bs; const float2* cot_sx; const float* cot_tc; long cot_tc_bs;
    int act;
    float res_scale;
    int gemm, gemm_tm;
    size_t partial_floats;
    int tile, pair;
    const void* wpb; const void* wph;
    int poly;
    int pool2; float* pool_tmp; long pool_tmp_bs;
    const void* wqb; const void* wqh;
};

enum PolyKind : int { POLY_UP = 0, POLY_ZINS_PAD2 = 1, POLY_ZINS_PAD1 = 2 };
inline int polyphase_vcout(int C, int a, int b, int co) { return ((a * (C / 64) + co / 64) * 2 + b) * 64 + (co % 64); }
void polyphase_fold(int kind, int nin, int nout, const float* w, long so, long si, long st, float* out);
void polyphase_fold_in(int nin, int nout, const float* w, long so, long si, long st, float* out, int noutP);

void launch_conv(const ConvArgs& a, int taps, hipStream_t st);
void launch_conv_bf16x3(const ConvArgs& a, int taps, hipStream_t st);
void launch_conv_f16(const ConvArgs& a, int taps, hipStream_t st);
void launch_conv_splitk_reduce(const ConvArgs& a, hipStream_t st);

struct ConvEnv {
    int prec = 1;
    int chip_share = 1;
    int lanes = 1, lane_s0 = 0;
    float* partial = nullptr; size_t partial_floats = 0;
    float* stpart = nullptr; size_t stpart_floats = 0;
    bool fuse_stats = true, fuse_lin = true, deep1 = true;
    int max_batch = 1;
};

struct StatAsk {
    int kind = ST_NONE;
    bool norm = false;
    const float2* sx = nullptr;
    const float* prim = nullptr;
    float* keep = nullptr; size_t keep_floats = 0;
};

enum StatRoute : int {
    SR_NONE = 0,
    SR_EPI = 1,
    SR_SPLITK = 2,
    SR_ALONE = 3,
    SR_KEEP = 4,
};

struct ConvLaunch {
    ConvArgs args;
    int s0 = 0;
    int stats = SR_NONE;
    int ntile = 0;
};

struct ConvPlan {
    bool sc_first = false;
    int nl = 1;
    ConvLaunch l[2];
    bool stats_all = false;
    int keep_ntile = 0;
    bool pool_after = false; float* pool_out = nullptr; long pool_out_bs = 0; int pool_acc = 0;
    bool cot = false;
};

ConvPlan plan_conv(const ConvEnv& env, const ConvArgs& a, int taps, const StatAsk* ask, const ConvArgs* shortcut);
void conv_plan_family(ConvArgs& a, int prec);
void conv_plan_tile_pair(ConvArgs& a, int prec, int tile_override);

int conv_bf16_tile_couts(const ConvArgs& a);
const char* conv_variant_name(const ConvArgs& a, int taps, int prec);

void launch_fill_random(float* p, long count, unsigned seed, float scale, hipStream_t st);
void launch_gn_cache(const float* x, int C, int HW, int cpg, const float* sc, const float* sh, const float* mr,
                     float2* sx, hipStream_t st, int act = 0);

struct GemmArgs {
    const float* A; long sam, sak, sab;
    const float* Bm; long sbk, sbn, sbb;
    float* C; long scm, scn, scb;
    const float* bias;
    const float* colbias;
    const float* R; long srb;
    int M, N, K, batch;
    float alpha, beta;
    int batch2; long sah, sbh, sch;
    const float* A2; long sab2; const float* Bm2; long sbb2;
};
void launch_gemm(const GemmArgs& g, hipStream_t st);
void launch_gemm_pair(const GemmArgs& g0, const GemmArgs& g1, hipStream_t st);
enum GemmAct : int { GEMM_ACT_NONE = 0, GEMM_ACT_QUICK_GELU = 1, GEMM_ACT_GELU = 2, GEMM_ACT_RELU = 3 };
void launch_gemm_fixed(const GemmArgs& g, int act, hipStream_t st);
void launch_gemm_bf16x3(const GemmArgs& g, hipStream_t st);
bool gemm_prefers_bf16x3(const GemmArgs& g);
bool gemm_rec_eligible(const GemmArgs& g);
size_t gemm_rec_ws_bytes(const GemmArgs& g);
void launch_gemm_rec(const GemmArgs& g, unsigned char* ws, hipStream_t st);
enum GemmF32Variant : int { GEMM_F32_64 = 0, GEMM_F32_SMALL = 1, GEMM_F32_SMALL_PIPE = 2 };
int  gemm_f32_variant(const GemmArgs& g);
bool gemm_pair_grouped(const GemmArgs& g0, const GemmArgs& g1);
int  gemm_bf16x3_tile(const GemmArgs& g);
struct GemmRecRoute { int tm, ksplit, z[4], kcontig[4]; };
GemmRecRoute gemm_rec_route(const GemmArgs& g);

struct AttnFlashArgs {
    int T, NH, B, CH; float scale;
    const float *q, *k, *v; long hs;
    const float* P;
    const float* o;
    const float *dq, *dk, *dv; long bs_d;
    float* out; long bs_out;
    const float* go; long bs_go;
    float *gq, *gk, *gv; long bs_g;
    float* delta;
    int Lt; const float *kt, *vt;
    unsigned char* ws; size_t ws_bytes;
};
size_t attn_flash_ws_bytes(const AttnFlashArgs& a);
inline bool attn_flash_dma_route(const unsigned char* ws, size_t ws_bytes, size_t need, bool dma_on) {
    return ws != nullptr && dma_on && need <= ws_bytes;
}
bool attn_flash_dma_enabled();
bool attn_flash_supported(int T, int CH);
// ... 6 lines not shown
void launch_ln_tan(const float* dx, long dbs, const float* xprim, const float* sprim, int B, int C, int T, const float* gamma,
                   float* dy, long ybs, hipStream_t st);
void launch_ln_cot(const float* gy, long gbs, const float* xprim, const float* sprim, int B, int C, int T, const float* gamma,
                   const float* base, long base_bs, float* gx, long xbs, hipStream_t st);
struct XAttnArgs {
    int T, NH, B, CH, L, Lp, fwd;
    float alpha;
    const float* X; long x_bs;
    const float* K1; const float* K2;
    float* P; long p_bs;
    float* O; long o_bs;
};
bool xattn_fused_supported(int T, int CH, int L, int Lp);
void launch_xattn_fused(const XAttnArgs& a, hipStream_t st);
int  xattn_lg(int L);
struct XCtxArgs {
    int T, NH, B, CH, L, Lp;
    int walk, nchunk;
    float alpha;
    const float* go; long go_bs;
    const float* q;
    const float* V;
    const float* P;
    float* part;
    float* out; long out_bs;
};
bool xattn_ctx_supported(int T, int CH, int L, int Lp);
int  xattn_ctx_width(int L);
int  xattn_ctx_walk(int T, int NH, int CH, int L, int probes, size_t avail_floats);
void launch_xattn_ctx(const XCtxArgs& a, hipStream_t st);
void launch_geglu(int kind, const float* in, long in_bs, const float* fprim, int B, long n4, float* out, long out_bs,
                  hipStream_t st);

void launch_gn_stats(const float* x, long bs, int B, int C, int HW, int G, float eps,
                     const float* gamma, const float* beta,
                     float* mr, float* sc, float* sh, long stats_bs, double* scratch, hipStream_t st,
                     const float* ss_scale = nullptr, const float* ss_shift = nullptr);
void launch_gn_fused_finalize_cat(const float* partA, int C1, int ntA, const float* partB, int ntB, int B, int C, int HW, int G,
                                  float eps, const float* gamma, const float* beta, float* mr, float* sc, float* sh,
                                  long stats_bs, hipStream_t st);
void launch_gn_fused_finalize(const float* part, int ntile, int B, int C, int HW, int G, float eps, const float* gamma,
                              const float* beta, float* mr, float* sc, float* sh, long stats_bs, const float* ss_scale,
                              const float* ss_shift, hipStream_t st);
void launch_gn_lin_fused_finalize(int kind, const float* partA, int C1, int ntA, const float* partB, int ntB, int B, int C, int HW,
                                  int G, const float* mr, float* tst, float* tc, long tst_bs, hipStream_t st);
void launch_conv_splitk_reduce_stats(const ConvArgs& a, int kind, int G, float eps, const float* gamma, const float* beta,
                                     float* mr, float* sc, float* sh, long stats_bs, const float* ss_scale,
                                     const float* ss_shift, const float* prim, const float* sc_prim, const float* sh_prim,
                                     const float* mr_prim, float* tst, float* tc, long tst_bs, double* scratch,
                                     hipStream_t st);
void launch_gn_tstats(const float* d, long d_bs, const float* x, long x_bs, int B, int C, int HW, int G,
                      const float* sc, const float* sh, const float* mr, long pbs_c, long pbs_g,
                      int kind, float* tst, float* tc, long tst_bs, double* scratch, hipStream_t st, int act = 0);
void launch_gn_apply(int kind, const float* d, long d_bs, const float* x, long x_bs,
                     const float* base, long base_bs, float* out, long out_bs, int accumulate,
                     int B, int C, int HW, int G, const float* sc, const float* sh, const float* mr,
                     long pbs_c, long pbs_g, const float* tst, long tst_bs, hipStream_t st, int act = 0,
                     float base_scale = 1.0f);

void launch_ctx_groupnorm(const float* tok, int L, int D, int G, float eps, const float* gamma, const float* beta,
                          float* out, hipStream_t st);

void launch_softmax_rows(float* S, long rows, int T, hipStream_t st, int B = 1, long bs = 0);
void launch_softmax_jac(float* dS, const float* P, long rows, int T, long p_rows, float scale, hipStream_t st,
                        int B = 1, long bs = 0);

void launch_temb(float t, int ch, int temb_ch, const float* freq, const float* w0, const float* b0,
                 const float* w1, const float* b1, float* scratch, hipStream_t st, int cos_first = 0,
                 const float* add = nullptr,
                 const float* t_ptr = nullptr,
                 int act = 0,
                 const float* add_in = nullptr);
void launch_set_scalar(float* p, float v, hipStream_t st);
void launch_clock_stamp(unsigned long long* out2, hipStream_t st);
void launch_temb_proj(const float* tact, int temb_ch, const float* w, const float* b, int cout,
                      float* out, hipStream_t st);
void launch_pool2x2_sum(const float* in, long in_bs, float* out, long out_bs, int accumulate,
                        int B, int C, int Hout, int Wout, hipStream_t st, float scale = 1.0f);
void launch_upsample2x(const float* in, long in_bs, float* out, long out_bs, int accumulate, float scale, int B,
                       int C, int Hin, int Win, hipStream_t st);
void launch_copy(const float* in, long in_bs, float* out, long out_bs, int accumulate,
                 int B, long per_sample, hipStream_t st);
void launch_add_rows(const float* in, long in_bs, const float* add, long add_bs, float scale, float* out, long out_bs, int B,
                     long per_sample, hipStream_t st);
void launch_zero_rows(float* out, long out_bs, int B, long per_sample, hipStream_t st);

void launch_ddim_step(const float* x, const float* eps, const float* noise, float* out, float* x0_out, long count,
                      float c_x0_x, float c_x0_e, float c_next_x0, float c_next_e, float c_noise,
                      hipStream_t st);
void launch_asym_step(const float* x, const float* eps_edit, const float* eps_src, float* out, float* x0_out, long count, float c_x0_x,
                      float c_x0_e, float c_next_x0, float c_next_e, hipStream_t st);
void launch_latent_sample(const float* mom, const float* noise, float scale, float* z, int B, long zhw, hipStream_t st);
void launch_masked_axpby(const float* V, const float* dE, const uint8_t* mask, float cv, float ce,
                         float* U, int k, long n, hipStream_t st, const uint8_t* mask2 = nullptr, long split = 0);
void launch_cot_seed(const float* U, const uint8_t* mask, float cv, float ce, float* gE, float* gX0,
                     int k, long n, hipStream_t st, const uint8_t* mask2 = nullptr, long split = 0);
void launch_add(const float* a, const float* b, float* out, long count, hipStream_t st);
void launch_lincomb(const float* const* src, const float* coef, int n, float* out, long count, hipStream_t st);
void launch_diffedit_mask(const float* eps_a, const float* eps_b, float scale, int B, int C, long HW, int rule, float* m,
                          uint8_t* mask, float* part, float* status, hipStream_t st);
void launch_cfg_masked_step(const float* x, const float* ef, const float* ee, const float* en, const uint8_t* mask, float* out,
                            int B, long n, float g, float c_x0_x, float c_x0_e, float c_next_x0, float c_next_e,
                            hipStream_t st);
void launch_lcm_step(const float* x, const float* eps, const float* noise, float* prev, float* den, long count, float sat,
                     float s1mat, float satp, float s1matp, float c_skip, float c_out, hipStream_t st);

void launch_gram(const float* A, int k, long n, double* G, double* scratch, hipStream_t st, const double* gate = nullptr);
void launch_cross_gram(const float* A, int k1, const float* B, int k2, long n, double* C, double* scratch,
                       hipStream_t st, const double* gate = nullptr);
constexpr int SOLVER_W_GATE = 64;
constexpr double SOLVER_W_FLOOR = 0x1p-47;
constexpr double SOLVER_REORTHO_RATIO = 1e-7;
void launch_jacobi_eig(double* G, int k, double* w, double* Q, hipStream_t st);
void launch_rotate_rows(const float* Ain, float* Aout, int k, long n, const double* Q, const double* w,
                        int mode, hipStream_t st);
void launch_sign_fix(float* A, int k, long n, float* s_out, const double* w, float* scratch, hipStream_t st,
                     double* sign_out = nullptr);
void launch_cholesky(double* G, int k, hipStream_t st, double drop_below = 0.0, double* w = nullptr,
                     const double* gate = nullptr);
void launch_trsm_rows(const float* Ain, float* Aout, int k, long n, const double* L, hipStream_t st,
                      const double* gate = nullptr);
void launch_convergence(const float* a, const float* b, long count, float atol, float rtol, float* out2,
                        double* scratch, hipStream_t st);
void launch_convergence_rows(const float* a, const float* b, int k, long n, float atol, float rtol, float* out2,
                             double* scratch, hipStream_t st);
void launch_project_rows(const float* Vm, int k, const float* Vn, int k0, long n, const double* C,
                         float* out, hipStream_t st);
void launch_normalize_rows(float* A, int k, long n, double* scratch, hipStream_t st);
constexpr int KRYLOV_MAX_BLOCK = 32;
constexpr double KRYLOV_DROP = 1e-6;
constexpr int KRY_T = 0;
constexpr int KRY_W = KRY_T + 64 * 64;
constexpr int KRY_THETA = KRY_W + 64 * 64;
constexpr int KRY_G = KRY_THETA + 72;
constexpr int KRY_SIGN = KRY_G + KRYLOV_MAX_BLOCK * KRYLOV_MAX_BLOCK;
constexpr int KRY_STATE = KRY_SIGN + KRYLOV_MAX_BLOCK;
void launch_krylov_fill_t(const double* Ct, int m, int k, double* T, double* Tp, hipStream_t st);
void launch_rotate_rect(const float* Q, float* out, int k, int m, long n, const double* W, int ldw, const double* sign,
                        hipStream_t st);
void launch_krylov_resid(const double* W, int m, int k, const double* G, const double* theta, float* resid, float* stat,
                         int has_prev, hipStream_t st);
void launch_krylov_floor(double* w, int k, const double* theta, float* stat, hipStream_t st);
void launch_row_sqnorm(const float* A, int k, long n, float* s, double* scratch, hipStream_t st);
void launch_edit_axpy(const float* x, const float* v, const float* alphas_dev, int B, long n, float* out,
                      hipStream_t st);
void launch_mask_gather(const float* U, const int* idx, long L, long n, int k, float* out, hipStream_t st);
void launch_mask_compact(const uint8_t* mask, long n, int* idx, int* count, hipStream_t st);

}
```

### loco-edit_amd/csrc/misc.hip

```cpp
#include "kernels.h"

namespace loco {

typedef float f32x4_t __attribute__((ext_vector_type(4)));

__device__ __forceinline__ double wave_sum(double v) {
#pragma unroll
    for (int o = 32; o > 0; o >>= 1) v += __shfl_down(v, o, 64);
    return v;
}
__device__ __forceinline__ float wave_sumf(float v) {
#pragma unroll
    for (int o = 32; o > 0; o >>= 1) v += __shfl_down(v, o, 64);
    return v;
}
__device__ __forceinline__ float wave_maxf(float v) {
#pragma unroll
    for (int o = 32; o > 0; o >>= 1) v = fmaxf(v, __shfl_down(v, o, 64));
    return v;
}
__device__ __forceinline__ double block_sum(double v, double* sm) {
    v = wave_sum(v);
    __syncthreads();
    if ((threadIdx.x & 63) == 0) sm[threadIdx.x >> 6] = v;
    __syncthreads();
    double r = 0.0;
    for (int i = 0; i < (int)(blockDim.x >> 6); ++i) r += sm[i];
    return r;
}

__global__ __launch_bounds__(256) void gn_partial_kernel(const float* x, long bs, long len, double* scratch) {
    __shared__ double sm[4];
    const int s = blockIdx.x, nsplit = gridDim.x, g = blockIdx.y, b = blockIdx.z, G = gridDim.y;
    const float* p = x + (long)b * bs + (long)g * len;
    long per = ((len / 4 + nsplit - 1) / nsplit) * 4;
    long beg = (long)s * per, end = beg + per < len ? beg + per : len;
    if (beg > end) beg = end;
    const long n4 = (end - beg) / 4;
    const float4* p4 = reinterpret_cast<const float4*>(p + beg);
    double sum = 0.0;
    for (long i = threadIdx.x; i < n4; i += 256) {
        float4 v = p4[i];
        sum += (double)((v.x + v.y) + (v.z + v.w));
    }
    for (long i = beg + n4 * 4 + threadIdx.x; i < end; i += 256) sum += (double)p[i];
    double tot = block_sum(sum, sm);
    const double cnt = (double)(end - beg);
    const float mean = cnt > 0 ? (float)(tot / cnt) : 0.f;
    double m2 = 0.0;
    for (long i = threadIdx.x; i < n4; i += 256) {
        float4 v = p4[i];
        float a0 = v.x - mean, a1 = v.y - mean, a2 = v.z - mean, a3 = v.w - mean;
        m2 += (double)((a0 * a0 + a1 * a1) + (a2 * a2 + a3 * a3));
// ... 429 lines not shown
            float aa = gm * rstd, oo = beta[c] - meanf * rstd * gm;
            if (ss_scale) {
                const float f = 1.0f + ss_scale[c];
                aa *= f;
                oo = oo * f + ss_shift[c];
            }
            sc[(long)b * sbs + c] = aa;
            sh[(long)b * sbs + c] = oo;
        }
    } else {
        const float m1 = (float)(t1 * inv_n), m2 = (float)(t2 * inv_n);
        if (threadIdx.x == 0) {
            tst[(long)b * tbs + 2 * g] = m1;
            tst[(long)b * tbs + 2 * g + 1] = m2;
        }
        if (tc && threadIdx.x < cpg) {
            const float f = KIND == ST_TAN ? 1.0f : rstd_p;
            float* t = tc + (long)b * tbs + 2 * ((long)g * cpg + threadIdx.x);
            t[0] = f * m1;
            t[1] = f * m2;
        }
    }
}

void launch_conv_splitk_reduce_stats(const ConvArgs& a, int kind, int G, float eps, const float* gamma, const float* beta,
                                     float* mr, float* sc, float* sh, long stats_bs, const float* ss_scale,
                                     const float* ss_shift, const float* prim, const float* sc_prim, const float* sh_prim,
                                     const float* mr_prim, float* tst, float* tc, long tst_bs, double* scratch,
                                     hipStream_t st) {
    const int HW = a.Hout * a.Wout, cpg = a.Cout / G;
    const long len = (long)cpg * HW;
    const int ns = gn_nsplit(len, a.B * G);
    dim3 grid(ns, G, a.B);
    long pieces = (len / ns + 3) / 4;
    int nthr = (int)((pieces + 63) / 64) * 64;
    if (nthr < 64) nthr = 64;
    if (nthr > 1024) nthr = 1024;
    if (nthr < cpg) nthr = ((cpg + 63) / 64) * 64;
#define RS(K) hipLaunchKernelGGL(splitk_reduce_stats_kernel<K>, grid, dim3(nthr), 0, st, a, G, eps, gamma, beta, mr, sc, sh, \
                                 stats_bs, ss_scale, ss_shift, prim, sc_prim, sh_prim, mr_prim, tst, tc, tst_bs, scratch)
    if (kind == ST_FWD) RS(ST_FWD); else if (kind == ST_TAN) RS(ST_TAN); else RS(ST_COT);
#undef RS
    if (ns == 1) return;
    if (kind == ST_FWD) {
        hipLaunchKernelGGL(gn_finalize_kernel, dim3((G + 63) / 64, a.B), dim3(64), 0, st, scratch, ns, G, a.Cout, eps, gamma,
                           beta, mr, sc, sh, stats_bs, ss_scale, ss_shift);
    } else {
        const long BG = (long)a.B * G;
        hipLaunchKernelGGL(gn_tstats_finalize, dim3((unsigned)((BG + 255) / 256)), dim3(256), 0, st, scratch, ns, BG, G,
                           1.0 / (double)len, tst, tc, tst_bs, cpg, mr_prim, 0L, kind == ST_TAN ? 0 : 1);
    }
}

template <int KIND>
__global__ __launch_bounds__(256) void gn_apply_kernel(const float* d, long d_bs, const float* x, long x_bs,
                                                       const float* base, long base_bs, float* out, long out_bs,
                                                       int accumulate, int C, int HW, int cpg, const float* sc,
                                                       const float* sh, const float* mr, long pbs_c, long pbs_g,
                                                       const float* tst, long tbs, int act, float base_scale) {
    const int b = blockIdx.y;
    const long per = (long)C * HW;
    for (long i = ((long)blockIdx.x * 256 + threadIdx.x) * 4; i < per; i += (long)gridDim.x * 1024) {
        int c = (int)(i / HW);
        int g = c / cpg;
        float scc = sc[(long)b * pbs_c + c], shc = sh[(long)b * pbs_c + c];
        float4 xv = *reinterpret_cast<const float4*>(x + (long)b * x_bs + i);
        float xx[4] = {xv.x, xv.y, xv.z, xv.w};
        float r[4];
        if (KIND == 0) {
#pragma unroll
            for (int j = 0; j < 4; ++j) r[j] = fmaf(scc, xx[j], shc);
        } else if (KIND == 4) {
#pragma unroll
            for (int j = 0; j < 4; ++j) r[j] = act_fwd(fmaf(scc, xx[j], shc), act);
        } else {
            float mean = mr[(long)b * pbs_g + 2 * g], rstd = mr[(long)b * pbs_g + 2 * g + 1];
            float m1 = tst[(long)b * tbs + g * 2], m2 = tst[(long)b * tbs + g * 2 + 1];
            float4 dv = *reinterpret_cast<const float4*>(d + (long)b * d_bs + i);
            float dd[4] = {dv.x, dv.y, dv.z, dv.w};
            float bb[4] = {0.f, 0.f, 0.f, 0.f};
            if (KIND >= 2 && base) {
                float4 bv = *reinterpret_cast<const float4*>(base + (long)b * base_bs + i);
                bb[0] = base_scale * bv.x; bb[1] = base_scale * bv.y; bb[2] = base_scale * bv.z; bb[3] = base_scale * bv.w;
            }
            float gm = scc / rstd;
#pragma unroll
            for (int j = 0; j < 4; ++j) {
                float xh = (xx[j] - mean) * rstd;
                if (KIND == 1) r[j] = scc * (dd[j] - m1 - xh * m2);
                else if (KIND == 5) r[j] = act_der(fmaf(scc, xx[j], shc), act) * scc * (dd[j] - m1 - xh * m2);
                else if (KIND == 2) r[j] = bb[j] + rstd * (gm * act_der(fmaf(scc, xx[j], shc), act) * dd[j] - m1 - xh * m2);
                else r[j] = bb[j] + rstd * (gm * dd[j] - m1 - xh * m2);
            }
        }
        float4* o = reinterpret_cast<float4*>(out + (long)b * out_bs + i);
        if (accumulate) {
            float4 ov = *o;
            r[0] += ov.x; r[1] += ov.y; r[2] += ov.z; r[3] += ov.w;
        }
        *o = make_float4(r[0], r[1], r[2], r[3]);
    }
}

void launch_gn_apply(int kind, const float* d, long d_bs, const float* x, long x_bs, const float* base,
                     long base_bs, float* out, long out_bs, int accumulate, int B, int C, int HW, int G,
                     const float* sc, const float* sh, const float* mr, long pbs_c, long pbs_g, const float* tst,
                     long tst_bs, hipStream_t st, int act, float base_scale) {
    long per = (long)C * HW;
    int blocks = (int)((per / 4 + 255) / 256);
    if (blocks > 1024) blocks = 1024;
    dim3 grid(blocks, B);
    int cpg = C / G;
#define GA(K) hipLaunchKernelGGL(gn_apply_kernel<K>, grid, dim3(256), 0, st, d, d_bs, x, x_bs, base, base_bs, out, \
                                 out_bs, accumulate, C, HW, cpg, sc, sh, mr, pbs_c, pbs_g, tst, tst_bs, act, base_scale)
    switch (kind) {
        case 0: GA(0); break;
        case 1: GA(1); break;
        case 2: GA(2); break;
        case 4: GA(4); break;
        case 5: GA(5); break;
        default: GA(3); break;
    }
#undef GA
}

__global__ __launch_bounds__(256) void gn_cache_kernel(const float* x, int C, int HW, int cpg, const float* sc,
                                                       const float* sh, const float* mr, float2* sx, int act) {
    const long per = (long)C * HW;
    for (long i = ((long)blockIdx.x * 256 + threadIdx.x) * 4; i < per; i += (long)gridDim.x * 1024) {
        int c = (int)(i / HW);
        int g = c / cpg;
        float scc = sc[c], shc = sh[c], mean = mr[2 * g], rstd = mr[2 * g + 1];
        float4 xv = *reinterpret_cast<const float4*>(x + i);
        float xx[4] = {xv.x, xv.y, xv.z, xv.w};
        float4 o0, o1;
        float r[8];
#pragma unroll
        for (int j = 0; j < 4; ++j) {
            r[2 * j] = scc * act_der(fmaf(scc, xx[j], shc), act);
            r[2 * j + 1] = (xx[j] - mean) * rstd;
        }
        o0 = make_float4(r[0], r[1], r[2], r[3]);
        o1 = make_float4(r[4], r[5], r[6], r[7]);
        float4* o = reinterpret_cast<float4*>(sx + i);
        o[0] = o0;
        o[1] = o1;
    }
}
void launch_gn_cache(const float* x, int C, int HW, int cpg, const float* sc, const float* sh, const float* mr,
                     float2* sx, hipStream_t st, int act) {
    long per = (long)C * HW;
    int blocks = (int)((per / 4 + 255) / 256);
    if (blocks > 2048) blocks = 2048;
    hipLaunchKernelGGL(gn_cache_kernel, dim3(blocks), dim3(256), 0, st, x, C, HW, cpg, sc, sh, mr, sx, act);
}

__global__ __launch_bounds__(256) void ctx_groupnorm_kernel(const float* tok, int L, int D, int cpg, float eps,
                                                            const float* gamma, const float* beta, float* out) {
    __shared__ double sm[4];
    const int g = blockIdx.x, n = L * cpg;
    double s1 = 0.0;
    for (int i = threadIdx.x; i < n; i += 256) s1 += (double)tok[(long)(i / cpg) * D + g * cpg + (i % cpg)];
    const double mean = block_sum(s1, sm) / (double)n;
    __syncthreads();
    double s2 = 0.0;
    for (int i = threadIdx.x; i < n; i += 256) {
        const double d = (double)tok[(long)(i / cpg) * D + g * cpg + (i % cpg)] - mean;
        s2 += d * d;
    }
    const double var = block_sum(s2, sm) / (double)n;
    const float mf = (float)mean, rstd = (float)(1.0 / sqrt(var + (double)eps));
// ... 240 lines not shown
        *reinterpret_cast<float4*>(out + (long)b * out_bs + i) = make_float4(0.f, 0.f, 0.f, 0.f);
}
void launch_zero_rows(float* out, long out_bs, int B, long per_sample, hipStream_t st) {
    int blocks = (int)((per_sample / 4 + 255) / 256);
    if (blocks > 2048) blocks = 2048;
    if (blocks < 1) blocks = 1;
    hipLaunchKernelGGL(zero_rows_kernel, dim3(blocks, B), dim3(256), 0, st, out, out_bs, per_sample);
}

__global__ void ddim_step_kernel(const float* x, const float* eps, const float* noise, float* out, float* x0_out,
                                 long count, float sq1mat, float sqat, float sqatn, float ce, float cn) {
    for (long i = (long)blockIdx.x * blockDim.x + threadIdx.x; i < count; i += (long)gridDim.x * blockDim.x) {
        float e = eps[i];
        float p = (x[i] - e * sq1mat) / sqat;
        float v = sqatn * p + ce * e;
        if (noise) v += cn * noise[i];
        if (x0_out) x0_out[i] = p;
        out[i] = v;
    }
}
void launch_ddim_step(const float* x, const float* eps, const float* noise, float* out, float* x0_out, long count,
                      float c_x0_x, float c_x0_e, float c_next_x0, float c_next_e, float c_noise, hipStream_t st) {
    int blocks = (int)((count + 255) / 256);
    if (blocks > 2048) blocks = 2048;
    hipLaunchKernelGGL(ddim_step_kernel, dim3(blocks), dim3(256), 0, st, x, eps, noise, out, x0_out, count, c_x0_e, c_x0_x,
                       c_next_x0, c_next_e, c_noise);
}

__global__ void asym_step_kernel(const float* x, const float* eps_edit, const float* eps_src, float* out, float* x0_out, long count,
                                 float sq1mat, float sqat, float sqatn, float ce) {
    for (long i = (long)blockIdx.x * blockDim.x + threadIdx.x; i < count; i += (long)gridDim.x * blockDim.x) {
        const float p = __fdiv_rn(fmaf(-sq1mat, eps_edit[i], x[i]), sqat);
        if (x0_out) x0_out[i] = p;
        out[i] = __fadd_rn(__fmul_rn(ce, eps_src[i]), __fmul_rn(sqatn, p));
    }
}
void launch_asym_step(const float* x, const float* eps_edit, const float* eps_src, float* out, float* x0_out, long count, float c_x0_x,
                      float c_x0_e, float c_next_x0, float c_next_e, hipStream_t st) {
    int blocks = (int)((count + 255) / 256);
    if (blocks > 2048) blocks = 2048;
    hipLaunchKernelGGL(asym_step_kernel, dim3(blocks), dim3(256), 0, st, x, eps_edit, eps_src, out, x0_out, count, c_x0_e, c_x0_x, c_next_x0,
                       c_next_e);
}

__global__ void masked_axpby_kernel(const float* V, const float* dE, const uint8_t* mask, float cv, float ce,
                                    float* U, long n, long total, const uint8_t* mask2, long split) {
    for (long i = (long)blockIdx.x * blockDim.x + threadIdx.x; i < total; i += (long)gridDim.x * blockDim.x) {
        long row = i / n, j = i - row * n;
        const uint8_t* mk = (mask2 && row >= split) ? mask2 : mask;
        const bool pass = !mk || mk[j];
        U[i] = pass ? ((V ? cv * V[i] : 0.f) + ce * dE[i]) : 0.f;
    }
}
void launch_masked_axpby(const float* V, const float* dE, const uint8_t* mask, float cv, float ce, float* U, int k,
                         long n, hipStream_t st, const uint8_t* mask2, long split) {
    long total = (long)k * n;
    int blocks = (int)((total + 255) / 256);
    if (blocks > 4096) blocks = 4096;
    hipLaunchKernelGGL(masked_axpby_kernel, dim3(blocks), dim3(256), 0, st, V, dE, mask, cv, ce, U, n, total, mask2, split);
}

__global__ void latent_sample_kernel(const float* mom, const float* noise, float scale, float* z, long zhw, long total) {
    for (long i = (long)blockIdx.x * blockDim.x + threadIdx.x; i < total; i += (long)gridDim.x * blockDim.x) {
        const long b = i / zhw, j = i - b * zhw;
        const float mean = mom[b * 2 * zhw + j];
        const float lv = fminf(fmaxf(mom[b * 2 * zhw + zhw + j], -30.f), 20.f);
        z[i] = scale * (mean + expf(0.5f * lv) * (noise ? noise[i] : 0.f));
    }
}
void launch_latent_sample(const float* mom, const float* noise, float scale, float* z, int B, long zhw, hipStream_t st) {
    const long total = (long)B * zhw;
    int blocks = (int)((total + 255) / 256);
    if (blocks > 2048) blocks = 2048;
    hipLaunchKernelGGL(latent_sample_kernel, dim3(blocks), dim3(256), 0, st, mom, noise, scale, z, zhw, total);
}

__global__ void cot_seed_kernel(const float* U, const uint8_t* mask, float cv, float ce, float* gE, float* gX0,
                                long n, long total, const uint8_t* mask2, long split) {
    for (long i = (long)blockIdx.x * blockDim.x + threadIdx.x; i < total; i += (long)gridDim.x * blockDim.x) {
        long row = i / n, j = i - row * n;
        const uint8_t* mk = (mask2 && row >= split) ? mask2 : mask;
        float u = (!mk || mk[j]) ? U[i] : 0.f;
        gE[i] = ce * u;
        if (gX0) gX0[i] = cv * u;
    }
}
void launch_cot_seed(const float* U, const uint8_t* mask, float cv, float ce, float* gE, float* gX0, int k, long n,
                     hipStream_t st, const uint8_t* mask2, long split) {
    long total = (long)k * n;
    int blocks = (int)((total + 255) / 256);
    if (blocks > 4096) blocks = 4096;
    hipLaunchKernelGGL(cot_seed_kernel, dim3(blocks), dim3(256), 0, st, U, mask, cv, ce, gE, gX0, n, total, mask2, split);
}

__global__ void fill_random_kernel(float* p, long count, unsigned seed, float scale) {
    for (long i = (long)blockIdx.x * blockDim.x + threadIdx.x; i < count; i += (long)gridDim.x * blockDim.x) {
        unsigned h = (unsigned)i * 2654435761u + seed;
        h ^= h >> 16; h *= 0x85ebca6bu; h ^= h >> 13; h *= 0xc2b2ae35u; h ^= h >> 16;
        p[i] = scale * ((float)(h & 0xFFFFFF) / 8388608.0f - 1.0f);
    }
}
void launch_fill_random(float* p, long count, unsigned seed, float scale, hipStream_t st) {
    hipLaunchKernelGGL(fill_random_kernel, dim3(2048), dim3(256), 0, st, p, count, seed, scale);
}

struct LinComb { const float* src[4]; float coef[4]; int n; };
// ... 41 lines not shown
```

### loco-edit_amd/hip.py

```python
from __future__ import annotations

import ctypes as C
import os
from typing import Dict, Optional

import numpy as np
import torch

from .config import UNetConfig

_LIB_PATH = os.environ.get("LOCO_HIP_LIB") or os.path.join(os.path.dirname(os.path.abspath(__file__)), "libloco_hip.so")
_lib = None

DIAG_SYMBOLS = ["loco_bench_conv", "loco_debug_conv", "loco_debug_attn", "loco_debug_norm", "loco_debug_gemm", "loco_debug_pointwise",
                "loco_debug_tensor"]

SYMBOLS = [
    "loco_version", "loco_device_count", "loco_create", "loco_fork", "loco_destroy", "loco_last_error",
    "loco_load_param", "loco_params_missing", "loco_unet_forward", "loco_ddim_step", "loco_sched_step",
    "loco_pmp_primal", "loco_pmp_set_second_mask", "loco_pmp_jvp", "loco_pmp_vjp", "loco_pmp_vjp_context", "loco_orthonormalize", "loco_qr_rows",
    "loco_convergence", "loco_convergence_rows", "loco_krylov_extend", "loco_krylov_ritz", "loco_krylov_left", "loco_null_project", "loco_edit_axpy", "loco_mask_gather", "loco_mask_count",
    "loco_unet_flops", "loco_workspace_bytes", "loco_clock_stamp", "loco_set_side_stream", "loco_timer_start", "loco_timer_stop",
    "loco_profile_enable", "loco_profile_report", "loco_set_precision", "loco_get_precision", "loco_set_streams", "loco_set_chip_share",
    "loco_set_cond", "loco_set_context", "loco_lincomb", "loco_masked_axpby", "loco_latent_sample",
    "loco_text_create", "loco_text_load_param", "loco_text_params_missing", "loco_text_encode", "loco_text_last_error",
    "loco_text_destroy", "loco_t5_create", "loco_text_encode_masked",
    "loco_diffedit_mask", "loco_cfg_masked_step", "loco_set_time_cond", "loco_lcm_step",
    "loco_h_dims", "loco_unet_get_h", "loco_unet_forward_dh", "loco_pmp_primal_tap", "loco_pmp_primal_eps", "loco_pmp_primal_tap_dh", "loco_sched_step_asym",
    "loco_sam_create", "loco_sam_load_param", "loco_sam_params_missing", "loco_sam_encode", "loco_sam_profile",
    "loco_sam_profile_read", "loco_sam_last_error", "loco_sam_destroy",
    "loco_samdec_create", "loco_samdec_load_param", "loco_samdec_params_missing", "loco_samdec_set_image", "loco_samdec_predict",
    "loco_samdec_score", "loco_samdec_binarize", "loco_samdec_last_error", "loco_samdec_destroy",
    "loco_clipvis_create", "loco_clipvis_load_param", "loco_clipvis_params_missing", "loco_clipvis_preprocess",
    "loco_clipvis_encode", "loco_clipvis_last_error", "loco_clipvis_destroy",
    "loco_clipvis_enable_grad", "loco_clipvis_grad_bytes", "loco_clipvis_encode_vjp", "loco_clipvis_preprocess_f32",
    "loco_clipvis_preprocess_f32_vjp", "loco_clipvis_encode_taps",
    "loco_clipseg_create", "loco_clipseg_load_param", "loco_clipseg_params_missing", "loco_clipseg_logit_size", "loco_clipseg_decode",
    "loco_clipseg_preprocess", "loco_clipseg_masks", "loco_clipseg_last_error", "loco_clipseg_destroy",
    "loco_quality_create", "loco_quality_load_param", "loco_quality_params_missing", "loco_quality_lpips", "loco_quality_ssim",
    "loco_quality_masked_mse", "loco_quality_last_error", "loco_quality_destroy",
    "loco_pca_create", "loco_pca_reset", "loco_pca_rows", "loco_pca_add_rows", "loco_pca_fit", "loco_pca_center", "loco_pca_gram",
    "loco_pca_project", "loco_pca_set_route", "loco_pca_routes", "loco_pca_last_error", "loco_pca_destroy",
    "loco_asyrp_create", "loco_asyrp_load_param", "loco_asyrp_params_missing", "loco_asyrp_read_param", "loco_asyrp_read_grad",
    "loco_asyrp_forward", "loco_asyrp_backward", "loco_asyrp_zero_grad", "loco_asyrp_adam_step", "loco_asyrp_reset_moments",
    "loco_asyrp_last_error", "loco_asyrp_destroy",
]

TAPS = {None: 0, "enc": 1, "dec": 2}

DIFFEDIT_RULES = {"reference": 0, "intended": 1}


class LocoCfg(C.Structure):
    _fields_ = [
        ("struct_size", C.c_int32), ("resolution", C.c_int32), ("in_channels", C.c_int32), ("out_ch", C.c_int32), ("ch", C.c_int32),
        ("num_levels", C.c_int32), ("ch_mult", C.c_int32 * 8), ("num_res_blocks", C.c_int32),
        ("num_attn_res", C.c_int32), ("attn_resolutions", C.c_int32 * 8), ("gn_groups", C.c_int32),
        ("gn_eps", C.c_float), ("max_batch", C.c_int32),
        ("arch", C.c_int32), ("num_head_channels", C.c_int32), ("learn_sigma", C.c_int32),
        ("context_dim", C.c_int32), ("context_len", C.c_int32),
        ("scale_shift_norm", C.c_int32), ("resblock_updown", C.c_int32), ("num_heads", C.c_int32),
        ("transformer_depth", C.c_int32),
        ("act", C.c_int32), ("res_scale", C.c_float), ("added_kv", C.c_int32),
        ("time_cond_proj_dim", C.c_int32),
    ]


class LocoConvDesc(C.Structure):
# ... 242 lines not shown
        lib.loco_clipseg_preprocess.argtypes = [vp, vp, i32, i32, i32, i32, i32, i32, C.POINTER(C.c_float), C.POINTER(C.c_float), vp, vp]
        lib.loco_clipseg_masks.argtypes = [vp, vp, i32, i32, i32, C.c_double, vp, vp, vp]
        lib.loco_clipseg_last_error.argtypes = [vp]
        lib.loco_clipseg_last_error.restype = C.c_char_p
        lib.loco_clipseg_destroy.argtypes = [vp]
        lib.loco_clipseg_destroy.restype = None
    if hasattr(lib, "loco_quality_create"):
        lib.loco_quality_create.argtypes = [C.POINTER(LocoQualityCfg), i32, i32, C.POINTER(vp)]
        lib.loco_quality_load_param.argtypes = [vp, C.c_char_p, vp, C.POINTER(i64), i32]
        lib.loco_quality_params_missing.argtypes = [vp]
        lib.loco_quality_lpips.argtypes = [vp, vp, vp, i32, i32, i32, i32, vp, vp, vp]
        lib.loco_quality_ssim.argtypes = [vp, vp, vp, i32, i32, i32, i32, C.c_double, vp, vp]
        lib.loco_quality_masked_mse.argtypes = [vp, vp, vp, vp, i32, i64, vp, vp, vp]
        lib.loco_quality_last_error.argtypes = [vp]
        lib.loco_quality_last_error.restype = C.c_char_p
        lib.loco_quality_destroy.argtypes = [vp]
        lib.loco_quality_destroy.restype = None
    if hasattr(lib, "loco_pca_create"):
        lib.loco_pca_create.argtypes = [i32, i64, i64, i32, C.POINTER(vp)]
        lib.loco_pca_reset.argtypes = [vp]
        lib.loco_pca_rows.argtypes = [vp]
        lib.loco_pca_rows.restype = i64
        lib.loco_pca_add_rows.argtypes = [vp, vp, i64, i64, vp]
        lib.loco_pca_fit.argtypes = [vp, i32, i32, vp, i32, vp, vp, vp, vp]
        lib.loco_pca_center.argtypes = [vp, i32, vp, vp, vp]
        lib.loco_pca_gram.argtypes = [vp, vp, i64, i32, vp, vp]
        lib.loco_pca_project.argtypes = [vp, vp, i32, i32, i32, vp, vp]
        lib.loco_pca_set_route.argtypes = [vp, i32]
        lib.loco_pca_routes.argtypes = [vp]
        lib.loco_pca_routes.restype = C.c_char_p
        lib.loco_pca_last_error.argtypes = [vp]
        lib.loco_pca_last_error.restype = C.c_char_p
        lib.loco_pca_destroy.argtypes = [vp]
        lib.loco_pca_destroy.restype = None
    if hasattr(lib, "loco_asyrp_create"):
        lib.loco_asyrp_create.argtypes = [i32, i32, i32, i32, i32, i32, f32, C.POINTER(vp)]
        lib.loco_asyrp_load_param.argtypes = [vp, C.c_char_p, vp, C.POINTER(i64), i32]
        lib.loco_asyrp_params_missing.argtypes = [vp]
        lib.loco_asyrp_read_param.argtypes = [vp, C.c_char_p, vp, i64]
        lib.loco_asyrp_read_grad.argtypes = [vp, C.c_char_p, vp, i64]
        lib.loco_asyrp_forward.argtypes = [vp, vp, vp, i32, f32, vp, i32, vp]
        lib.loco_asyrp_backward.argtypes = [vp, vp, i32, vp, vp]
        lib.loco_asyrp_zero_grad.argtypes = [vp, vp]
        lib.loco_asyrp_adam_step.argtypes = [vp, f32, f32, f32, f32, i32, vp]
        lib.loco_asyrp_reset_moments.argtypes = [vp, vp]
        lib.loco_asyrp_last_error.argtypes = [vp]
        lib.loco_asyrp_last_error.restype = C.c_char_p
        lib.loco_asyrp_destroy.argtypes = [vp]
        lib.loco_asyrp_destroy.restype = None
    if hasattr(lib, "loco_bench_conv"):
        lib.loco_bench_conv.argtypes = [vp, i32, i32, i32, i32, i32, i32, i32, i32, i32, C.POINTER(f32), vp]
        lib.loco_debug_tensor.argtypes = [vp, C.c_char_p, vp, i64, vp]
        lib.loco_debug_tensor.restype = i64
    if hasattr(lib, "loco_debug_conv"):
        lib.loco_debug_conv.argtypes = [vp, C.POINTER(LocoConvDesc), C.c_char_p, i64, vp]
    if hasattr(lib, "loco_debug_attn"):
        lib.loco_debug_attn.argtypes = [vp, C.POINTER(LocoAttnDesc), C.c_char_p, i64, vp]
    if hasattr(lib, "loco_debug_norm"):
        lib.loco_debug_norm.argtypes = [vp, C.POINTER(LocoNormDesc), vp]
    if hasattr(lib, "loco_debug_pointwise"):
        lib.loco_debug_pointwise.argtypes = [vp, C.POINTER(LocoPointwiseDesc), vp]
    if hasattr(lib, "loco_debug_gemm"):
        lib.loco_debug_gemm.argtypes = [vp, C.POINTER(LocoGemmDesc), C.c_char_p, i64, vp]
    _lib = lib
    return lib


def _ptr(t: Optional[torch.Tensor]):
    return None if t is None else C.c_void_p(t.data_ptr())


def _stream():
    return C.c_void_p(torch.cuda.current_stream().cuda_stream)


def _chk_dev(t: torch.Tensor, dtype=torch.float32):
    if not t.is_cuda:
        raise ValueError("loco_hip operates on device tensors only")
    if t.dtype != dtype:
        raise ValueError(f"expected {dtype}, got {t.dtype}")
    if not t.is_contiguous():
        raise ValueError("tensor must be contiguous")


def c_cfg(cfg: UNetConfig, max_batch: int) -> LocoCfg:
    c = LocoCfg()
    c.struct_size = C.sizeof(LocoCfg)
    c.resolution, c.in_channels, c.out_ch, c.ch = cfg.resolution, cfg.in_channels, cfg.out_ch, cfg.ch
    c.num_levels = len(cfg.ch_mult)
    for i, m in enumerate(cfg.ch_mult):
        c.ch_mult[i] = m
    c.num_res_blocks = cfg.num_res_blocks
    c.num_attn_res = len(cfg.attn_resolutions)
    for i, r in enumerate(cfg.attn_resolutions):
        c.attn_resolutions[i] = r
    c.gn_groups, c.gn_eps, c.max_batch = cfg.gn_groups, cfg.gn_eps, int(max_batch)
    c.arch = {"ddpm": 0, "adm": 1, "dec": 2, "enc": 3}[cfg.arch]
    c.num_head_channels, c.learn_sigma = cfg.num_head_channels, int(cfg.learn_sigma)
    c.context_dim, c.context_len = cfg.context_dim, cfg.context_len
    c.scale_shift_norm, c.resblock_updown = int(cfg.scale_shift_norm), int(cfg.resblock_updown)
    c.num_heads, c.transformer_depth = cfg.num_heads, cfg.transformer_depth
    c.act, c.res_scale, c.added_kv = {"silu": 0, "gelu": 1}[cfg.act], float(cfg.res_scale), int(cfg.added_kv)
    c.time_cond_proj_dim = int(cfg.time_cond_proj_dim)
    return c


# ... 451 lines not shown
    def sclk_mhz(stamp0: torch.Tensor, stamp1: torch.Tensor) -> float:
        d = (stamp1 - stamp0).tolist()
        return 100.0 * d[0] / max(d[1], 1)

    def unet_flops(self) -> float:
        return float(self.lib.loco_unet_flops(self._ctx))

    def workspace_bytes(self) -> int:
        return int(self.lib.loco_workspace_bytes(self._ctx))

    def timer_start(self):
        self._check(self.lib.loco_timer_start(self._ctx, _stream()), "loco_timer_start")

    def timer_stop(self) -> float:
        ms = C.c_float()
        self._check(self.lib.loco_timer_stop(self._ctx, _stream(), C.byref(ms)), "loco_timer_stop")
        return float(ms.value)

    PRECISIONS = {"f32": 0, "bf16x3": 1, "f16": 2}

    def set_precision(self, mode: str):
        self._check(self.lib.loco_set_precision(self._ctx, self.PRECISIONS[mode]), "loco_set_precision")

    def set_streams(self, n: int):
        self._check(self.lib.loco_set_streams(self._ctx, int(n)), "loco_set_streams")

    def set_chip_share(self, n: int):
        self._check(self.lib.loco_set_chip_share(self._ctx, int(n)), "loco_set_chip_share")

    def set_side_stream(self, stream: "Optional[torch.cuda.Stream]"):
        self._side_stream = stream
        ptr = C.c_void_p(stream.cuda_stream) if stream is not None else None
        self._check(self.lib.loco_set_side_stream(self._ctx, ptr), "loco_set_side_stream")

    def set_streams_measured(self, n: int):
        if n == 2:
            from .tloco import BranchStreams
            side = BranchStreams._pick(1, self.device)
            if not side:
                self.set_streams(1)
                return 1
            self.set_side_stream(side[0])
        self.set_streams(n)
        return n

    def get_precision(self) -> str:
        m = self.lib.loco_get_precision(self._ctx)
        return {v: k for k, v in self.PRECISIONS.items()}[m]

    def _need_diag(self, sym):
        if not hasattr(self.lib, sym):
            raise RuntimeError(f"{sym} is a diagnostic of include/loco_hip_diag.h: build `make -C loco-edit_amd/csrc diag` "
                               "and set LOCO_HIP_LIB=<repo>/loco-edit_amd/libloco_hip_diag.so")

    def bench_conv(self, cin, cout, H, W, B, mode, taps=9, tile=-1, iters=20) -> float:
        self._need_diag("loco_bench_conv")
        ms = C.c_float()
        self._check(self.lib.loco_bench_conv(self._ctx, cin, cout, H, W, B, mode, taps, tile, iters, C.byref(ms),
                                             _stream()), "loco_bench_conv")
        return float(ms.value)

    def debug_conv(self, out: torch.Tensor, with_closing: bool = False, **desc):
        self._need_diag("loco_debug_conv")
        d = LocoConvDesc()
        d.struct_size = C.sizeof(LocoConvDesc)
        d.stride, d.in_arena, d.pad, d.res_scale = 1, 1, -1, 1.0
        keep = []
        _chk_dev(out)
        d.out = out.data_ptr()
        for k, v in desc.items():
            if k not in LocoConvDesc._PTRS:
                if not hasattr(d, k) or k == "struct_size":
                    raise TypeError(f"debug_conv: no descriptor field {k!r}")
                setattr(d, k, v)
            elif v is not None:
                if k in LocoConvDesc._HOST:
                    v = v.detach().to("cpu", torch.float32).contiguous()
                else:
                    _chk_dev(v)
                keep.append(v)
                setattr(d, k, v.data_ptr())
        buf = C.create_string_buffer(1 << 12)
        rc = self.lib.loco_debug_conv(self._ctx, C.byref(d), buf, len(buf), _stream())
        if rc not in (0, 1):
            self._check(rc, "loco_debug_conv")
        plan = []
        closing = None
        for line in buf.value.decode().splitlines():
            rec = dict(f.split("=", 1) for f in line.split(" "))
            rec = {k: (v if k in ("kernel", "stats") else int(v)) for k, v in rec.items()}
            if "launch" in rec:
                plan.append(rec)
            else:
                closing = rec
        return (plan, rc == 0, closing) if with_closing else (plan, rc == 0)

    def debug_norm(self, op: str, **desc):
        self._need_diag("loco_debug_norm")
        d = LocoNormDesc()
        d.struct_size = C.sizeof(LocoNormDesc)
        d.op, d.base_scale, d.B = LocoNormDesc.OPS[op], 1.0, 1
        keep = []
        for k, v in desc.items():
            if k not in LocoNormDesc._PTRS:
                if not hasattr(d, k) or k in ("struct_size", "op"):
                    raise TypeError(f"debug_norm: no descriptor field {k!r}")
# ... 765 lines not shown
```

Baseline: 20.61 edit-directions/s.

## Skip masked-out spatial tiles in output conv tangent and cotangent passes

Builds per-tile liveness flags from the edit mask, dilated by one pixel for the input side. The final output conv of the tangent pass and the first conv of the cotangent pass then early-exit tiles that have no masked pixels. The cotangent path either zero-fills skipped tiles or skips writing them, in which case the following GN apply reads flags to treat them as zero. This cuts MFMA work on the 256x256 output convs, since the mask covers a small region, at the cost of new kernel variants, a mask-tile pre-pass, and correctness depending on the tile geometry and dilation logic.

```diff
diff --git a/include/loco_hip_diag.h b/include/loco_hip_diag.h
--- a/include/loco_hip_diag.h
+++ b/include/loco_hip_diag.h
@@ -97,6 +97,8 @@
 
 int64_t loco_debug_tensor(loco_ctx* ctx, const char* name, float* dst, int64_t cap, void* stream);
 
+int loco_debug_fill_tangent(loco_ctx* ctx, uint32_t bits, void* stream);
+
 #ifdef __cplusplus
 }
 #endif
diff --git a/loco-edit_amd/csrc/conv_bf16.hip b/loco-edit_amd/csrc/conv_bf16.hip
--- a/loco-edit_amd/csrc/conv_bf16.hip
+++ b/loco-edit_amd/csrc/conv_bf16.hip
@@ -11,6 +11,7 @@
 void launch_conv_gemm(const ConvArgs& a, hipStream_t st);
 template <int PR> void launch_poly_b(const ConvArgs& a, hipStream_t st);
 template <int PR> void launch_poly_in_b(const ConvArgs& a, hipStream_t st);
+template <int PR> void launch_mtile_b(const ConvArgs& a, hipStream_t st);
 
 template <int PR>
 static void launch_lowp(const ConvArgs& a, int taps, hipStream_t st) {
@@ -43,6 +44,7 @@
             return;
         }
     }
+    if (taps == 9 && a.mtile) { launch_mtile_b<PR>(a, st); return; }
     if (taps == 9) {
         switch (a.mode) {
             case CM_NONE: launch_tile_b<PR, 9, CM_NONE>(a, st); break;
diff --git a/loco-edit_amd/csrc/conv_bf16_inst_m.hip b/loco-edit_amd/csrc/conv_bf16_inst_m.hip
--- /dev/null
+++ b/loco-edit_amd/csrc/conv_bf16_inst_m.hip
@@ -0,0 +1,5 @@
+#include "conv_bf16_kernel.h"
+
+namespace loco {
+template void launch_mtile_b<PR_BF16X3>(const ConvArgs&, hipStream_t);
+}
diff --git a/loco-edit_amd/csrc/conv_bf16_inst_m_f16.hip b/loco-edit_amd/csrc/conv_bf16_inst_m_f16.hip
--- /dev/null
+++ b/loco-edit_amd/csrc/conv_bf16_inst_m_f16.hip
@@ -0,0 +1,5 @@
+#include "conv_bf16_kernel.h"
+
+namespace loco {
+template void launch_mtile_b<PR_F16>(const ConvArgs&, hipStream_t);
+}
diff --git a/loco-edit_amd/csrc/conv_bf16_kernel.h b/loco-edit_amd/csrc/conv_bf16_kernel.h
--- a/loco-edit_amd/csrc/conv_bf16_kernel.h
+++ b/loco-edit_amd/csrc/conv_bf16_kernel.h
@@ -465,7 +465,30 @@
     }
 }
 
-template <int PR, int TAPS, int WM, int WN, int TM, int TN, int MODE, int STG, int PHASE = 0>
+template <int NTHR, int MT, int NT>
+__device__ __forceinline__ void conv_lowp_zero_tile(const ConvArgs& a, const int co0, const int oy0, const int ox0, const int TW,
+                                                    const int tile_id, const int b) {
+    constexpr int NQ = NT / 4, RSTEP = NTHR / NQ;
+    static_assert(NTHR % NQ == 0 && MT <= NTHR && MT % RSTEP == 0, "zero tile: task rows");
+    const int tid = threadIdx.x;
+    if (a.st_part && tid < MT && co0 + tid < a.Cout) {
+        const int ntile = (a.Hout * a.Wout) / NT;
+        float* const sp = a.st_part + (long)b * a.Cout * ntile * 2;
+        *reinterpret_cast<f32x2*>(sp + ((long)(co0 + tid) * ntile + tile_id) * 2) = f32x2{0.f, 0.f};
+    }
+    if (a.mtile_mode == MTILE_ZERO) {
+        const int twsh = 31 - __builtin_clz((unsigned)TW);
+        const int row0 = tid / NQ, quad0 = tid & (NQ - 1);
+        const long out_plane = (long)a.Hout * a.Wout;
+        float* const ob = a.out + (long)b * a.out_bs + (long)(oy0 + ((quad0 * 4) >> twsh)) * a.Wout + ox0 + ((quad0 * 4) & (TW - 1));
+        const f32x4 z = {0.f, 0.f, 0.f, 0.f};
+#pragma unroll 4
+        for (int r = row0; r < MT; r += RSTEP)
+            if (co0 + r < a.Cout) __builtin_nontemporal_store(z, reinterpret_cast<f32x4*>(ob + (long)(co0 + r) * out_plane));
+    }
+}
+
+template <int PR, int TAPS, int WM, int WN, int TM, int TN, int MODE, int STG, int PHASE = 0, bool MSK = false>
 __device__ __forceinline__ void conv_lowp_body(const ConvArgs& a, f32x16 (&acc)[TM][TN]) {
     constexpr int NTHR = WM * WN * 64;
     constexpr int HP = halo_pitch<PR>();
@@ -544,6 +567,14 @@
     idivmod_small(zid, a.nsplit, zb_, zs_);
     const int b = __builtin_amdgcn_readfirstlane(zb_);
     const int split = __builtin_amdgcn_readfirstlane(zs_);
+
+    if constexpr (MSK) {
+        static_assert(PHASE == 0 && TAPS == 9, "mask tile flags: whole 3x3 launches");
+        if (__builtin_amdgcn_readfirstlane((int)a.mtile[tile_id]) == 0) {
+            if (a.mtile_mode != MTILE_SKIP) conv_lowp_zero_tile<NTHR, MT, NT>(a, co0, oy0, ox0, TW, tile_id, b);
+            return;
+        }
+    }
 
     if constexpr (XPF && PHASE != 2 && EARLY_W) {
         const int nchunks_ = (a.Cin + BKC - 1) / BKC;
@@ -1295,6 +1326,16 @@
     f32x16 acc[TM][TN];
     conv_lowp_body<PR_F16, TAPS, WM, WN, TM, TN, MODE, STG>(a, acc);
 }
+template <int TAPS, int WM, int WN, int TM, int TN, int MODE, int STG>
+__global__ __launch_bounds__(WM * WN * 64, lowp_min_waves(TAPS, WM * WN * 64)) void conv_mfma_bf16x3_mt(ConvArgs a) {
+    f32x16 acc[TM][TN];
+    conv_lowp_body<PR_BF16X3, TAPS, WM, WN, TM, TN, MODE, STG, 0, true>(a, acc);
+}
+template <int TAPS, int WM, int WN, int TM, int TN, int MODE, int STG>
+__global__ __launch_bounds__(WM * WN * 64, lowp_min_waves(TAPS, WM * WN * 64)) void conv_mfma_f16_mt(ConvArgs a) {
+    f32x16 acc[TM][TN];
+    conv_lowp_body<PR_F16, TAPS, WM, WN, TM, TN, MODE, STG, 0, true>(a, acc);
+}
 
 template <int PR, int WM, int WN, int TM, int TN, int MODE>
 __device__ __forceinline__ void conv_lowp_kcat(const ConvArgs& a) {
@@ -1309,7 +1350,7 @@
 template <int WM, int WN, int TM, int TN, int MODE>
 __global__ __launch_bounds__(WM * WN * 64) void conv_kcat_f16(ConvArgs a) { conv_lowp_kcat<PR_F16, WM, WN, TM, TN, MODE>(a); }
 
-template <int PR, int TAPS, int WM, int WN, int TM, int TN, int MODE, int STG>
+template <int PR, int TAPS, int WM, int WN, int TM, int TN, int MODE, int STG, bool MSK = false>
 static void launch_one_b2(const ConvArgs& a, hipStream_t st) {
     constexpr int MT = WM * TM * 32, NT = WN * TN * 32;
     constexpr int KS = (TAPS == 9) ? 3 : (TAPS == 4 ? 2 : 1), HK = (TAPS == 1) ? 1 : 3;
@@ -1322,7 +1363,9 @@
     if (lds < stage_bytes) lds = stage_bytes;
     dim3 grid(((a.Hout * a.Wout) / NT) * ((a.Cout + MT - 1) / MT) * a.B * a.nsplit);
     void (*kern)(ConvArgs);
-    if constexpr (PR == PR_F16) kern = &conv_mfma_f16<TAPS, WM, WN, TM, TN, MODE, STG>;
+    if constexpr (MSK && PR == PR_F16) kern = &conv_mfma_f16_mt<TAPS, WM, WN, TM, TN, MODE, STG>;
+    else if constexpr (MSK) kern = &conv_mfma_bf16x3_mt<TAPS, WM, WN, TM, TN, MODE, STG>;
+    else if constexpr (PR == PR_F16) kern = &conv_mfma_f16<TAPS, WM, WN, TM, TN, MODE, STG>;
     else kern = &conv_mfma_bf16x3<TAPS, WM, WN, TM, TN, MODE, STG>;
     if (lds > 64 * 1024) {
         static DeviceOnce once;
@@ -1381,6 +1424,12 @@
     launch_one_b2<PR, 4, 2, 4, 2, 2, CM_NONE, 1>(v, st);
 }
 
+template <int PR>
+void launch_mtile_b(const ConvArgs& a, hipStream_t st) {
+    if (a.mtile_mode == MTILE_SKIP) launch_one_b2<PR, 9, 1, 4, 1, 1, CM_TAN_SILU, 0, true>(a, st);
+    else launch_one_b2<PR, 9, 2, 4, 2, 2, CM_NONE, 1, true>(a, st);
+}
+
 template <int PR, int TAPS, int MODE>
 void launch_tile_b(const ConvArgs& a, hipStream_t st) {
     switch (a.tile) {
diff --git a/loco-edit_amd/csrc/conv_plan.hip b/loco-edit_amd/csrc/conv_plan.hip
--- a/loco-edit_amd/csrc/conv_plan.hip
+++ b/loco-edit_amd/csrc/conv_plan.hip
@@ -109,6 +109,31 @@
     return a.tile == 5;
 }
 
+int conv_mtile_pixels(int prec, int Cout, int H, int W, int B) {
+    if (prec < 1) return 0;
+    ConvArgs a{};
+    a.Cout = Cout; a.Hout = H; a.Wout = W; a.B = B; a.taps = 9; a.stride = 1; a.nsplit = 1;
+    return kNT[bf16_tile_of(a)];
+}
+
+static bool conv_mtile_ok(const ConvEnv& e, const ConvArgs& a, int taps, int tail, const StatAsk* q) {
+    if (e.prec < 1 || taps != 9 || a.nsplit != 1 || tail || a.gemm || a.poly || a.pool2 || a.Cin2 > 0) return false;
+    if (a.stride != 1 || a.upsample || a.zins || a.pad != 1 || a.Hin != a.Hout || a.Win != a.Wout) return false;
+    const int NT = kNT[a.tile], TW = a.Wout < 32 ? a.Wout : 32;
+    if (a.mtile_px != NT || (TW & (TW - 1)) != 0 || (TW % 4) != 0 || (NT % TW) != 0 || (a.Wout % TW) != 0 || (a.Hout % (NT / TW)) != 0) return false;
+    const bool general = (a.Cin % BKC) != 0 || !a.in_padded;
+    if (a.mtile_mode == MTILE_SKIP)
+        return a.mode == CM_TAN_SILU && a.tile == 2 && !general && !(q && q->kind != ST_NONE);
+    if (a.mtile_mode != MTILE_ZERO && a.mtile_mode != MTILE_ZERO_NOWRITE) return false;
+    return a.mode == CM_NONE && a.tile == 5 && general && (a.Cout % 128) == 0 && !a.bias && !a.bias2 && !a.res && !a.cot_d && !a.accumulate;
+}
+static bool conv_mtile_stats_ok(const ConvLaunch& l, const StatAsk* q) {
+    if (l.args.pair) return false;
+    if (l.args.mtile_mode == MTILE_SKIP) return true;
+    return l.stats == SR_EPI || (l.stats == SR_NONE && !(q && q->kind != ST_NONE));
+}
+static void conv_mtile_clear(ConvArgs& a) { a.mtile = nullptr; a.mtile_px = 0; a.mtile_mode = MTILE_NONE; }
+
 static ConvArgs conv_shift_batch(const ConvArgs& a, int nb) {
     ConvArgs t = a;
     t.B = a.B - nb;
@@ -274,8 +299,11 @@
     int split = 1;
     const int tail = e.prec >= 1 && a.nsplit == 1 && a.B >= 2 && !a.gemm && !a.poly ? tail_split(a, e.partial_floats, &split) : 0;
     const bool want = q && q->kind != ST_NONE && e.prec >= 1 && e.fuse_stats;
+    if (a.mtile && !conv_mtile_ok(e, a, taps, tail, q)) conv_mtile_clear(a);
     if (!tail) {
         p.l[0] = plan_launch(e, q, want, a, 0, a.B, &p.keep_ntile);
+        if (p.l[0].args.mtile && !conv_mtile_stats_ok(p.l[0], q)) conv_mtile_clear(p.l[0].args);
+        p.mtile = p.l[0].args.mtile ? p.l[0].args.mtile_mode : MTILE_NONE;
         return p;
     }
     const bool per_part = want && q->norm && (q->kind == ST_FWD || (e.fuse_lin && (a.Hout * a.Wout) % 4 == 0));
@@ -332,7 +360,7 @@
 
 const char* conv_variant_name(const ConvArgs& a, int taps, int prec) {
     static const char* tiles[6] = {"2,2,2,2", "4,1,1,2", "1,4,1,1", "2,2,1,1", "2,2,2,4", "2,4,2,2"};
-    static char names[3][2][6][6][56];
+    static char names[3][2][6][6][2][56];
     static char others[3][3][6][40];
     const int mode = (a.mode < 0 || a.mode > 5) ? 2 : a.mode;
     const char* other = nullptr;
@@ -355,9 +383,10 @@
     int m = mode;
     if (taps != 9 && m != CM_NONE) m = CM_GN;
     if (!prec && m == CM_GN_GELU) m = CM_GN_SILU;
-    char* n = names[prec][taps == 9 ? 0 : 1][t][m];
+    const int mt = a.mtile ? 1 : 0;
+    char* n = names[prec][taps == 9 ? 0 : 1][t][m][mt];
     static const char* kn[3] = {"conv_mfma_f32", "conv_mfma_bf16x3", "conv_mfma_f16"};
-    if (!n[0]) snprintf(n, 56, "%s<%d,%s,%d>", kn[prec], taps, tiles[t], m);
+    if (!n[0]) snprintf(n, 56, "%s%s<%d,%s,%d>", kn[prec], mt ? "_mt" : "", taps, tiles[t], m);
     return n;
 }
 
diff --git a/loco-edit_amd/csrc/conv_plan_text.h b/loco-edit_amd/csrc/conv_plan_text.h
--- a/loco-edit_amd/csrc/conv_plan_text.h
+++ b/loco-edit_amd/csrc/conv_plan_text.h
@@ -17,9 +17,9 @@
         const ConvArgs& y = l.args;
         snprintf(line, sizeof(line),
                  "launch=%d part=0 kernel=%s tile=%d nsplit=%d B=%d s0=%d gemm=%d gemm_tm=%d pair=%d Cin2=%d sc_first=%d cot=%d "
-                 "stats=%s ntile=%d\n",
+                 "stats=%s ntile=%d mtile=%d\n",
                  li, conv_variant_name(y, taps, prec), y.tile, y.nsplit, y.B, l.s0, y.gemm, y.gemm ? y.gemm_tm : 0, y.pair, y.Cin2,
-                 p.sc_first ? 1 : 0, p.cot ? 1 : 0, stat_route_name(l.stats), l.ntile);
+                 p.sc_first ? 1 : 0, p.cot ? 1 : 0, stat_route_name(l.stats), l.ntile, y.mtile ? y.mtile_mode : 0);
         out += line;
     }
     snprintf(line, sizeof(line), "stats_all=%d keep_ntile=%d\n", p.stats_all ? 1 : 0, p.keep_ntile);
diff --git a/loco-edit_amd/csrc/engine.hip b/loco-edit_amd/csrc/engine.hip
--- a/loco-edit_amd/csrc/engine.hip
+++ b/loco-edit_amd/csrc/engine.hip
@@ -7,6 +7,7 @@
 
 #include "conv_plan_text.h"
 #include "engine_internal.h"
+#include "mask_tiles.h"
 
 using namespace loco;
 using namespace loco::eng;
@@ -108,7 +109,7 @@
     }
 }
 
-bool run_conv(loco_ctx* c, const ConvArgs& a0, int taps, hipStream_t st, const StatReq* rq, const ConvArgs* second) {
+bool run_conv(loco_ctx* c, const ConvArgs& a0, int taps, hipStream_t st, const StatReq* rq, const ConvArgs* second, int* mtile_mode) {
     const size_t span = (size_t)c->cfg.max_batch * c->prog->per_sample;
     auto padded = [&](const float* p) { return (p >= c->arenaP && p < c->arenaP + span) || (p >= c->arenaT && p < c->arenaT + span); };
     ConvArgs a = a0, sc;
@@ -127,6 +128,7 @@
     }
     const ConvPlan p = plan_conv(e, a, taps, rq ? &q : nullptr, second ? &sc : nullptr);
     if (p.sc_first) run_conv(c, *second, 1, st);
+    if (mtile_mode) *mtile_mode = p.mtile;
     if (c->plan_log) conv_plan_text(p, taps, c->prec, *c->plan_log);
     if (rq && rq->kind != ST_NONE && rq->n) rq->n->ready = true;
     if (rq && rq->keep_ntile) *rq->keep_ntile = p.keep_ntile;
@@ -514,13 +516,13 @@
     n.ready = false;
 }
 void gn_lin_apply(const Pass& p, const NormP& n, int kind, const TView& d, const float* x, const float* base, float* out,
-                  int accumulate = 0, float base_scale = 1.0f) {
+                  int accumulate = 0, float base_scale = 1.0f, const GnTiles* tiles = nullptr) {
     loco_ctx* c = p.c;
     NS sp = nstats(c, c->statsP, n);
     NS stt = nstats(c, p.stats, n);
     launch_gn_apply(kind, d, d.bs, x, 0, base, base ? d.bs : 0, out, d.bs, accumulate, p.B, d.C, d.H * d.W, c->cfg.gn_groups,
                     sp.sc, sp.sh, sp.mr, 0, 0, stt.tst, c->prog->stats_per_sample, p.st, kind == 2 || kind == 5 ? c->cfg.act : 0,
-                    base_scale);
+                    base_scale, tiles);
 }
 void set_tan(loco_ctx* c, ConvArgs& a, const NormP& n, const float* prim) {
     NS sp = nstats(c, c->statsP, n);
@@ -674,6 +676,10 @@
     return 0;
 }
 
+bool mask_tiles_apply(const loco_ctx* c, const Op& op) {
+    return c->mask_tiles && c->has_mask && !c->has_mask2 && (c->tap == 0 || c->tap == 2) && op.out == c->prog->eps_t;
+}
+
 int tangent_pass(loco_ctx* c, const float* V, int B, hipStream_t st, int op_lo = 0, int op_hi = -1) {
     const loco_unet_cfg& cfg = c->cfg;
     const long PS = c->prog->per_sample;
@@ -786,6 +792,7 @@
                 need_tan_stats(p, op.n1, op.in);
                 ConvArgs a = conv_args(TT(op.in), op.conv, false, TT(op.out), B, 3);
                 set_tan(c, a, op.n1, TP(op.in));
+                if (mask_tiles_apply(c, op) && c->mtile_px_out) { a.mtile = c->mtile_out; a.mtile_px = c->mtile_px_out; a.mtile_mode = MTILE_SKIP; }
                 run_conv(c, a, 9, st);
                 break;
             }
@@ -813,13 +820,20 @@
         const int acc = op.in_is_skip ? 1 : 0;
         switch (op.kind) {
             case OP_OUT: {
-                const ConvArgs a = conv_args(GO(op), op.conv, true, TG(op.a1), B, 3);
+                ConvArgs a = conv_args(GO(op), op.conv, true, TG(op.a1), B, 3);
+                if (mask_tiles_apply(c, op) && c->mtile_px_in) {
+                    a.mtile = c->mtile_in; a.mtile_px = c->mtile_px_in;
+                    a.mtile_mode = c->mask_tiles >= 2 ? MTILE_ZERO_NOWRITE : MTILE_ZERO;
+                }
+                int mt = MTILE_NONE;
                 {
                     const StatReq rq = req_lin(c, ST_COT, &op.n1, TP(op.in));
-                    run_conv(c, a, 9, st, &rq);
+                    run_conv(c, a, 9, st, &rq, nullptr, &mt);
                     op.n1.ready = false;
                 }
-                gn_lin_apply(p, op.n1, 2, TG(op.a1), TP(op.in), nullptr, TG(op.in));
+                const int TW = to.W < 32 ? to.W : 32;
+                const GnTiles gt{c->mtile_in, to.W, TW, TW ? c->mtile_px_in / TW : 0};
+                gn_lin_apply(p, op.n1, 2, TG(op.a1), TP(op.in), nullptr, TG(op.in), 0, 1.0f, mt == MTILE_ZERO_NOWRITE ? &gt : nullptr);
                 break;
             }
             case OP_UP: {
@@ -1059,6 +1073,12 @@
         c->prec = (e && std::string(e) == "f32") ? 0 : (e && std::string(e) == "f16") ? 2 : 1;
     }
     if (dalloc(c, &c->mask2, (size_t)c->prog->n_out)) return -1;
+    {
+        const char* e = getenv("LOCO_MASK_TILES");
+        c->mask_tiles = e ? std::max(0, std::min(2, atoi(e))) : 2;
+        const size_t nt = (size_t)c->prog->n_out / 64 + 16;
+        if (dalloc(c, &c->mtile_out, nt) || dalloc(c, &c->mtile_in, nt)) return -1;
+    }
     if (dalloc(c, &c->mask, (size_t)c->prog->n_out) || dalloc(c, &c->mask_idx, (size_t)c->prog->n_out) ||
         dalloc(c, &c->mask_L_dev, 4)) return -1;
     HIPCHK(c, hipEventCreate(&c->ev0));
@@ -1361,6 +1381,23 @@
         launch_mask_compact(c->mask, c->prog->n_out, c->mask_idx, c->mask_L_dev, st);
         c->mask_L = -1;
         c->mask_stream = st;
+    }
+    c->mtile_px_out = c->mtile_px_in = 0;
+    if (mask && c->mask_tiles && tap != 1) {
+        const Tens& te = c->tens[c->prog->eps_t];
+        const int TW = te.W < 32 ? te.W : 32;
+        for (const Op& op : c->ops) {
+            if (op.kind != OP_OUT || op.out != c->prog->eps_t || (long)te.C * te.H * te.W != (long)c->prog->n_out) continue;
+            const int px_out = conv_mtile_pixels(c->prec, te.C, te.H, te.W, 2), px_in = conv_mtile_pixels(c->prec, c->tens[op.in].C, te.H, te.W, 2);
+            auto fits = [&](int px) {
+                return px > 0 && (px % TW) == 0 && mask_tile_geom_ok(MaskTileGeom{te.H, te.W, TW, px / TW}) && te.H * te.W / px <= c->prog->n_out / 64 + 1;
+            };
+            c->mtile_px_out = fits(px_out) ? px_out : 0;
+            c->mtile_px_in = fits(px_in) ? px_in : 0;
+            if (c->mtile_px_out || c->mtile_px_in)
+                launch_mask_tiles(c->mask, te.C, te.H, te.W, TW, c->mtile_px_out / TW, c->mtile_px_out ? c->mtile_out : nullptr,
+                                  c->mtile_px_in / TW, c->mtile_px_in ? c->mtile_in : nullptr, st);
+        }
     }
     HIPCHK(c, hipGetLastError());
     c->primal_ok = true;
diff --git a/loco-edit_amd/csrc/engine_diag.hip b/loco-edit_amd/csrc/engine_diag.hip
--- a/loco-edit_amd/csrc/engine_diag.hip
+++ b/loco-edit_amd/csrc/engine_diag.hip
@@ -754,4 +754,10 @@
     return -3;
 }
 
-}
+int loco_debug_fill_tangent(loco_ctx* c, uint32_t bits, void* stream) {
+    if (!c) return -2;
+    HIPCHK(c, hipMemsetD32Async((hipDeviceptr_t)c->arenaT, (int)bits, (size_t)c->cfg.max_batch * c->prog->per_sample, (hipStream_t)stream));
+    return 0;
+}
+
+}
diff --git a/loco-edit_amd/csrc/engine_internal.h b/loco-edit_amd/csrc/engine_internal.h
--- a/loco-edit_amd/csrc/engine_internal.h
+++ b/loco-edit_amd/csrc/engine_internal.h
@@ -141,6 +141,9 @@
     int* mask_L_dev = nullptr;
     long mask_L = 0;
     hipStream_t mask_stream = nullptr;
+    int mask_tiles = 2;
+    uint8_t *mtile_out = nullptr, *mtile_in = nullptr;
+    int mtile_px_out = 0, mtile_px_in = 0;
     int primal_B = 0;
     hipEvent_t ev0 = nullptr, ev1 = nullptr;
     int n_streams = 1;
@@ -246,7 +249,7 @@
     return a;
 }
 bool run_conv(loco_ctx* c, const ConvArgs& a0, int taps, hipStream_t st, const StatReq* rq = nullptr,
-              const ConvArgs* second = nullptr);
+              const ConvArgs* second = nullptr, int* mtile_mode = nullptr);
 
 struct XA {
     loco_ctx* c; hipStream_t st; int B; int C, T, NH, CH, L, Lp;
diff --git a/loco-edit_amd/csrc/kernels.h b/loco-edit_amd/csrc/kernels.h
--- a/loco-edit_amd/csrc/kernels.h
+++ b/loco-edit_amd/csrc/kernels.h
@@ -79,6 +79,13 @@
     int poly;
     int pool2; float* pool_tmp; long pool_tmp_bs;
     const void* wqb; const void* wqh;
+    const uint8_t* mtile; int mtile_px; int mtile_mode;
+};
+enum MaskTileMode : int {
+    MTILE_NONE = 0,
+    MTILE_SKIP = 1,
+    MTILE_ZERO = 2,
+    MTILE_ZERO_NOWRITE = 3,
 };
 
 enum PolyKind : int { POLY_UP = 0, POLY_ZINS_PAD2 = 1, POLY_ZINS_PAD1 = 2 };
@@ -132,6 +139,7 @@
     int keep_ntile = 0;
     bool pool_after = false; float* pool_out = nullptr; long pool_out_bs = 0; int pool_acc = 0;
     bool cot = false;
+    int mtile = MTILE_NONE;
 };
 
 ConvPlan plan_conv(const ConvEnv& env, const ConvArgs& a, int taps, const StatAsk* ask, const ConvArgs* shortcut);
@@ -139,6 +147,7 @@
 void conv_plan_tile_pair(ConvArgs& a, int prec, int tile_override);
 
 int conv_bf16_tile_couts(const ConvArgs& a);
+int conv_mtile_pixels(int prec, int Cout, int H, int W, int B);
 const char* conv_variant_name(const ConvArgs& a, int taps, int prec);
 
 void launch_fill_random(float* p, long count, unsigned seed, float scale, hipStream_t st);
@@ -251,11 +260,13 @@
 void launch_gn_tstats(const float* d, long d_bs, const float* x, long x_bs, int B, int C, int HW, int G,
                       const float* sc, const float* sh, const float* mr, long pbs_c, long pbs_g,
                       int kind, float* tst, float* tc, long tst_bs, double* scratch, hipStream_t st, int act = 0);
+struct GnTiles { const uint8_t* flags; int W, TW, TH; };
 void launch_gn_apply(int kind, const float* d, long d_bs, const float* x, long x_bs,
                      const float* base, long base_bs, float* out, long out_bs, int accumulate,
                      int B, int C, int HW, int G, const float* sc, const float* sh, const float* mr,
                      long pbs_c, long pbs_g, const float* tst, long tst_bs, hipStream_t st, int act = 0,
-                     float base_scale = 1.0f);
+                     float base_scale = 1.0f,
+                     const GnTiles* tiles = nullptr);
 
 void launch_ctx_groupnorm(const float* tok, int L, int D, int G, float eps, const float* gamma, const float* beta,
                           float* out, hipStream_t st);
@@ -345,5 +356,7 @@
                       hipStream_t st);
 void launch_mask_gather(const float* U, const int* idx, long L, long n, int k, float* out, hipStream_t st);
 void launch_mask_compact(const uint8_t* mask, long n, int* idx, int* count, hipStream_t st);
-
-}
+void launch_mask_tiles(const uint8_t* mask, int C, int H, int W, int TW, int TH_out, uint8_t* tile_out, int TH_in, uint8_t* tile_in,
+                       hipStream_t st);
+
+}
diff --git a/loco-edit_amd/csrc/mask_tiles.h b/loco-edit_amd/csrc/mask_tiles.h
--- /dev/null
+++ b/loco-edit_amd/csrc/mask_tiles.h
@@ -0,0 +1,26 @@
+#pragma once
+#include <stdint.h>
+
+#if defined(__HIPCC__)
+#define LOCO_MT_HD __host__ __device__
+#else
+#define LOCO_MT_HD
+#endif
+
+namespace loco {
+
+struct MaskTileGeom { int H, W, TW, TH; };
+LOCO_MT_HD inline bool mask_tile_geom_ok(const MaskTileGeom& g) {
+    return g.TW > 0 && g.TH > 0 && (g.TW & (g.TW - 1)) == 0 && (g.TW % 4) == 0 && (g.W % g.TW) == 0 && (g.H % g.TH) == 0;
+}
+LOCO_MT_HD inline int mask_tile_count(const MaskTileGeom& g) { return (g.H / g.TH) * (g.W / g.TW); }
+LOCO_MT_HD inline int mask_tile_of(const MaskTileGeom& g, int y, int x) { return (y / g.TH) * (g.W / g.TW) + x / g.TW; }
+LOCO_MT_HD inline void mask_tile_mark(const MaskTileGeom& g, int y, int x, int grow, uint8_t* flag) {
+    for (int dy = -grow; dy <= grow; ++dy)
+        for (int dx = -grow; dx <= grow; ++dx) {
+            const int yy = y + dy, xx = x + dx;
+            if (yy >= 0 && yy < g.H && xx >= 0 && xx < g.W) flag[mask_tile_of(g, yy, xx)] = 1;
+        }
+}
+
+}
diff --git a/loco-edit_amd/csrc/misc.hip b/loco-edit_amd/csrc/misc.hip
--- a/loco-edit_amd/csrc/misc.hip
+++ b/loco-edit_amd/csrc/misc.hip
@@ -1,4 +1,5 @@
 #include "kernels.h"
+#include "mask_tiles.h"
 
 namespace loco {
 
@@ -534,12 +535,12 @@
     }
 }
 
-template <int KIND>
+template <int KIND, bool MT = false>
 __global__ __launch_bounds__(256) void gn_apply_kernel(const float* d, long d_bs, const float* x, long x_bs,
                                                        const float* base, long base_bs, float* out, long out_bs,
                                                        int accumulate, int C, int HW, int cpg, const float* sc,
                                                        const float* sh, const float* mr, long pbs_c, long pbs_g,
-                                                       const float* tst, long tbs, int act, float base_scale) {
+                                                       const float* tst, long tbs, int act, float base_scale, GnTiles mt) {
     const int b = blockIdx.y;
     const long per = (long)C * HW;
     for (long i = ((long)blockIdx.x * 256 + threadIdx.x) * 4; i < per; i += (long)gridDim.x * 1024) {
@@ -558,7 +559,13 @@
         } else {
             float mean = mr[(long)b * pbs_g + 2 * g], rstd = mr[(long)b * pbs_g + 2 * g + 1];
             float m1 = tst[(long)b * tbs + g * 2], m2 = tst[(long)b * tbs + g * 2 + 1];
-            float4 dv = *reinterpret_cast<const float4*>(d + (long)b * d_bs + i);
+            float4 dv = make_float4(0.f, 0.f, 0.f, 0.f);
+            bool live = true;
+            if (MT) {
+                const int pix = (int)(i - (long)c * HW), py = pix / mt.W, px = pix - py * mt.W;
+                live = mt.flags[(py / mt.TH) * (mt.W / mt.TW) + px / mt.TW] != 0;
+            }
+            if (live) dv = *reinterpret_cast<const float4*>(d + (long)b * d_bs + i);
             float dd[4] = {dv.x, dv.y, dv.z, dv.w};
             float bb[4] = {0.f, 0.f, 0.f, 0.f};
             if (KIND >= 2 && base) {
@@ -587,18 +594,19 @@
 void launch_gn_apply(int kind, const float* d, long d_bs, const float* x, long x_bs, const float* base,
                      long base_bs, float* out, long out_bs, int accumulate, int B, int C, int HW, int G,
                      const float* sc, const float* sh, const float* mr, long pbs_c, long pbs_g, const float* tst,
-                     long tst_bs, hipStream_t st, int act, float base_scale) {
+                     long tst_bs, hipStream_t st, int act, float base_scale, const GnTiles* tiles) {
     long per = (long)C * HW;
     int blocks = (int)((per / 4 + 255) / 256);
     if (blocks > 1024) blocks = 1024;
     dim3 grid(blocks, B);
     int cpg = C / G;
-#define GA(K) hipLaunchKernelGGL(gn_apply_kernel<K>, grid, dim3(256), 0, st, d, d_bs, x, x_bs, base, base_bs, out, \
-                                 out_bs, accumulate, C, HW, cpg, sc, sh, mr, pbs_c, pbs_g, tst, tst_bs, act, base_scale)
+    const GnTiles mt = tiles ? *tiles : GnTiles{nullptr, 0, 0, 0};
+#define GA(...) hipLaunchKernelGGL((gn_apply_kernel<__VA_ARGS__>), grid, dim3(256), 0, st, d, d_bs, x, x_bs, base, base_bs, out, \
+                                   out_bs, accumulate, C, HW, cpg, sc, sh, mr, pbs_c, pbs_g, tst, tst_bs, act, base_scale, mt)
     switch (kind) {
         case 0: GA(0); break;
         case 1: GA(1); break;
-        case 2: GA(2); break;
+        case 2: if (mt.flags) GA(2, true); else GA(2); break;
         case 4: GA(4); break;
         case 5: GA(5); break;
         default: GA(3); break;
@@ -945,6 +953,26 @@
         U[i] = pass ? ((V ? cv * V[i] : 0.f) + ce * dE[i]) : 0.f;
     }
 }
+__global__ void mask_tiles_kernel(const uint8_t* mask, long n, MaskTileGeom g_out, uint8_t* tile_out, MaskTileGeom g_in, uint8_t* tile_in) {
+    const int hw = g_out.H * g_out.W;
+    for (long i = (long)blockIdx.x * blockDim.x + threadIdx.x; i < n; i += (long)gridDim.x * blockDim.x) {
+        if (!mask[i]) continue;
+        const int pix = (int)(i % hw), y = pix / g_out.W, x = pix - y * g_out.W;
+        if (tile_out) mask_tile_mark(g_out, y, x, 0, tile_out);
+        if (tile_in) mask_tile_mark(g_in, y, x, 1, tile_in);
+    }
+}
+void launch_mask_tiles(const uint8_t* mask, int C, int H, int W, int TW, int TH_out, uint8_t* tile_out, int TH_in, uint8_t* tile_in,
+                       hipStream_t st) {
+    const MaskTileGeom g_out{H, W, TW, TH_out}, g_in{H, W, TW, TH_in};
+    if (tile_out) (void)hipMemsetAsync(tile_out, 0, (size_t)mask_tile_count(g_out), st);
+    if (tile_in) (void)hipMemsetAsync(tile_in, 0, (size_t)mask_tile_count(g_in), st);
+    const long n = (long)C * H * W;
+    int blocks = (int)((n + 255) / 256);
+    if (blocks > 1024) blocks = 1024;
+    hipLaunchKernelGGL(mask_tiles_kernel, dim3(blocks), dim3(256), 0, st, mask, n, g_out, tile_out, g_in, tile_in);
+}
+
 void launch_masked_axpby(const float* V, const float* dE, const uint8_t* mask, float cv, float ce, float* U, int k,
                          long n, hipStream_t st, const uint8_t* mask2, long split) {
     long total = (long)k * n;
diff --git a/loco-edit_amd/hip.py b/loco-edit_amd/hip.py
--- a/loco-edit_amd/hip.py
+++ b/loco-edit_amd/hip.py
@@ -13,7 +13,7 @@
 _lib = None
 
 DIAG_SYMBOLS = ["loco_bench_conv", "loco_debug_conv", "loco_debug_attn", "loco_debug_norm", "loco_debug_gemm", "loco_debug_pointwise",
-                "loco_debug_tensor"]
+                "loco_debug_tensor", "loco_debug_fill_tangent"]
 
 SYMBOLS = [
     "loco_version", "loco_device_count", "loco_create", "loco_fork", "loco_destroy", "loco_last_error",
@@ -362,6 +362,8 @@
         lib.loco_bench_conv.argtypes = [vp, i32, i32, i32, i32, i32, i32, i32, i32, i32, C.POINTER(f32), vp]
         lib.loco_debug_tensor.argtypes = [vp, C.c_char_p, vp, i64, vp]
         lib.loco_debug_tensor.restype = i64
+    if hasattr(lib, "loco_debug_fill_tangent"):
+        lib.loco_debug_fill_tangent.argtypes = [vp, C.c_uint32, vp]
     if hasattr(lib, "loco_debug_conv"):
         lib.loco_debug_conv.argtypes = [vp, C.POINTER(LocoConvDesc), C.c_char_p, i64, vp]
     if hasattr(lib, "loco_debug_attn"):
@@ -919,6 +921,10 @@
         if not hasattr(self.lib, sym):
             raise RuntimeError(f"{sym} is a diagnostic of include/loco_hip_diag.h: build `make -C loco-edit_amd/csrc diag` "
                                "and set LOCO_HIP_LIB=<repo>/loco-edit_amd/libloco_hip_diag.so")
+
+    def debug_fill_tangent(self, bits: int = 0x7FC00000) -> None:
+        self._need_diag("loco_debug_fill_tangent")
+        self._check(self.lib.loco_debug_fill_tangent(self._ctx, bits, _stream()), "loco_debug_fill_tangent")
 
     def bench_conv(self, cin, cout, H, W, B, mode, taps=9, tile=-1, iters=20) -> float:
         self._need_diag("loco_bench_conv")
```

Result: no change. 20.79 edit-directions/s (median of 6 runs) (+0.9%).
